# zyang1580/PDA

Measured on AMD Instinct MI355X. Metric: users/sec full-catalogue top-K@50 (eval), higher is better.
Workload: dtype f32; 1 GPU; C3: synthetic 1000000 users x 200000 items, d=128, PDA condition ((elu+1)*pop^0.22) head, masked top-K@50; ranks_seen=1

## Files before the change

include/pda_hip_experimental.h:

```cpp
#ifndef PDA_HIP_EXPERIMENTAL_H
#define PDA_HIP_EXPERIMENTAL_H

#include "pda_hip.h"

#ifdef __cplusplus
extern "C" {
#endif

int pda_score_topk_huge_splits(int n_users_blk, int n_items_local, int d);

int pda_topk_kth_value(const uint64_t* keys, int n_splits, int n_users_blk, int K, int pos, float* out, void* stream);
int pda_topk_remap_items(uint64_t* keys, size_t n_keys, const int32_t* gid, int n_gid, void* stream);
int pda_topk_seed_bounds(const uint64_t* keys, int n_splits, int n_users_blk, int K, int m, float* bounds, void* stream);
int pda_topk_seed_counts(const uint64_t* keys, int n_splits, int n_users_blk, int K, const float* bounds, int n_thr, int32_t* counts,
                         void* stream);
int pda_topk_seed_pick(const float* bounds, const int32_t* counts, int n_thr, int n_users_blk, int K, float* seed, void* stream);
int pda_topk_seed_refine(const uint64_t* keys, int n_splits, int n_users_blk, int K, float* lo, float* hi, float* mid, int32_t* counts,
                         int mode, void* stream);
int pda_score_topk4_phase_f32(const float* U, const float* I_shard, const void* prep, const float* pop_shard, const int32_t* users,
                              int n_users_blk, int item_offset, int n_items_local, int d, const int64_t* hist_indptr,
                              const int32_t* hist_indices, int hist_row_mode, int K, int head, int early_stop, int n_splits,
                              int phase, int warm_tiles, const float* seed, uint64_t* out_keys, void* workspace, void* stream);
int pda_score_topk4_phase_bf16(const uint16_t* U, const uint16_t* I_shard, const void* prep, const float* pop_shard,
                               const int32_t* users, int n_users_blk, int item_offset, int n_items_local, int d,
                               const int64_t* hist_indptr, const int32_t* hist_indices, int hist_row_mode, int K, int head,
                               int early_stop, int n_splits, int phase, int warm_tiles, const float* seed, uint64_t* out_keys,
                               void* workspace, void* stream);
int pda_score_topk4_phase_image_offsets(int n_users_blk, int n_items_local, int d, int n_splits, size_t* offs);
int pda_score_topk4_phase_user_image(const void* U, int bf16, const int32_t* users, int n_users_blk, int d, void* ufrag, float* unorm,
                                     void* stream);
int pda_score_topk4_phase_mask_table(const void* prep, int n_items_local, int d, int item_offset, const int64_t* hist_indptr,
                                     const int32_t* hist_indices, int n_rows, uint32_t* table, void* stream);
int pda_score_topk4_phase_masked_f32(const float* U, const float* I_shard, const void* prep, const float* pop_shard, const int32_t* users,
                                     int n_users_blk, int item_offset, int n_items_local, int d, const int64_t* hist_indptr,
                                     const int32_t* hist_indices, int hist_row_mode, int K, int head, int early_stop, int n_splits,
                                     const uint32_t* mask_table, int mask_table_rows, uint64_t* out_keys, void* workspace, void* stream);
int pda_score_topk4_phase_masked_bf16(const uint16_t* U, const uint16_t* I_shard, const void* prep, const float* pop_shard, const int32_t* users,
                                      int n_users_blk, int item_offset, int n_items_local, int d, const int64_t* hist_indptr,
                                      const int32_t* hist_indices, int hist_row_mode, int K, int head, int early_stop, int n_splits,
                                      const uint32_t* mask_table, int mask_table_rows, uint64_t* out_keys, void* workspace, void* stream);
int pda_score_topk4_phase_mask_rows(const void* prep, const int32_t* users, int n_users_blk, int item_offset, int n_items_local, int d,
                                    const int64_t* hist_indptr, const int32_t* hist_indices, int hist_row_mode, int warm_tiles, uint32_t* out,
                                    void* stream);
int pda_score_topk4_phase_mask_offsets(int n_users_blk, int n_items_local, int d, int n_splits, size_t* offs);
int pda_score_topk7_phase_user_image(const void* U, int bf16, const int32_t* users, int n_users_blk, int d, void* ufrag, float* unorm, float* uerr,
                                     void* stream);
int pda_score_topk4_phase_bloom_rows(const void* prep, const int32_t* users, int n_users_blk, const int64_t* hist_indptr,
                                     const int32_t* hist_indices, int hist_row_mode, int skip_if_ordered, uint32_t* bloom, void* stream);
int pda_score_topk7_phase_bloom_rows(const void* prep, const int32_t* users, int n_users_blk, int item_offset, int n_items_local, int d,
                                     const int64_t* hist_indptr, const int32_t* hist_indices, int hist_row_mode, uint32_t* bloom, void* stream);
#define PDA_SWEEP_WARM_ONE_KERNEL 2048
#define PDA_SWEEP_TAIL_NO_SHARE 4096
#define PDA_SWEEP_TAIL_OTHERS_FIRST 8192
#define PDA_SWEEP_TAIL_MIN2 16384

size_t pda_triplet_plan_bytes(int B);
size_t pda_triplet_plan_large_workspace_bytes(int B);
int pda_triplet_plan_large(const int32_t* users, const int32_t* pos, const int32_t* neg, int B, void* plan, void* workspace, void* stream);
size_t pda_bpr_step_plan_scratch_bytes(int B, int d);
int pda_triplet_plan(const int32_t* users, const int32_t* pos, const int32_t* neg, int B, int n_batches, void* plans, void* stream);
int pda_bpr_step_plan_f32(float* U, float* I, const int32_t* users, const int32_t* pos, const int32_t* neg, const float* pos_pop,
                          const float* neg_pop, int B, int d, float regs, float reg_div, float lr, const void* plan, float* scratch,
                          int exact, float* loss_acc, void* stream);
int pda_bpr_step_plan_bf16(uint16_t* U_bf16, uint16_t* I_bf16, float* U_master, float* I_master, const int32_t* users,
                           const int32_t* pos, const int32_t* neg, const float* pos_pop, const float* neg_pop, int B, int d,
                           float regs, float reg_div, float lr, const void* plan, float* scratch, float* loss_acc, void* stream);

int pda_sort_triplets_by_pos(int32_t* users, int32_t* pos, int32_t* neg, float* pos_pop, float* neg_pop, int B,
                             void* stream);

int pda_group_triplets_by_pos(int32_t* users, int32_t* pos, int32_t* neg, float* pos_pop, float* neg_pop, int B,
                              void* stream);

int pda_adam_mark_rows(const int32_t* users, const int32_t* pos, const int32_t* neg, int B, uint32_t* touched_u, uint32_t* touched_i, void* stream);
int pda_adam_dense_sweep3_f32(float* var_a, float* m_a, float* v_a, float* g_a, size_t rows_a, uint32_t* touched_a, float* var_b, float* m_b, float* v_b,
                              float* g_b, size_t rows_b, uint32_t* touched_b, int d, float lr_t, float beta1, float beta2, float eps, void* stream);

int pda_adam_rows_f32(float* var, float* m, float* v, float* g, const int32_t* rows, int n_rows, int d, float lr_t,
                      float beta1, float beta2, float eps, void* stream);

int pda_adam_lazy_f32(int phase, float* U, float* mU, float* vU, float* gU, int32_t* lastU, float* I, float* mI, float* vI,
                      float* gI, int32_t* lastI, const int32_t* users, const int32_t* pos, const int32_t* neg, int B, int d, int t,
                      const float* lr_tab, float beta1, float beta2, float eps, void* stream);
int pda_adam_lazy_sync_f32(float* var, float* m, float* v, int32_t* last, size_t n_rows, int d, int t, const float* lr_tab,
                           float beta1, float beta2, float eps, void* stream);
int pda_adam_lazy_dev_f32(int phase, float* U, float* mU, float* vU, float* gU, int32_t* lastU, float* I, float* mI, float* vI,
                          float* gI, int32_t* lastI, const int32_t* users, const int32_t* pos, const int32_t* neg, int B, int d,
                          const int32_t* t_dev, int32_t* t_next, const float* lr_tab, int n_tab, float beta1, float beta2, float eps,
                          void* stream);
#define PDA_ADAM_REPLAY_FAST 0x10
int pda_adam_lazy_sync_fast_f32(float* var, float* m, float* v, int32_t* last, size_t n_rows, int d, int t, const float* lr_tab,
                                float beta1, float beta2, float eps, void* stream);

typedef struct pda_sample_job {
    int32_t* users; int gen_users; const int32_t* user_pool; int n_pool; int B;
    const int64_t* train_indptr; const int32_t* train_indices; const int32_t* train_slots;
    int neg_lo, neg_hi; const float* pop_matrix; int n_slots; uint64_t seed;
    const uint64_t* step_dev; uint64_t* step_next;
    int32_t* pos; int32_t* neg; float* pos_pop; float* neg_pop;
} pda_sample_job;
int pda_bpr_step_sample_f32(float* U, float* I, const int32_t* users, const int32_t* pos, const int32_t* neg,
                            const float* pos_pop, const float* neg_pop, int B, int d, float regs, float reg_div, float lr,
                            int update_mode, float* loss_acc, const pda_sample_job* next, void* stream);

int pda_sample_batches_dev(int32_t* users, int gen_users, const int32_t* user_pool, int n_pool, int B, int n_batches,
                           const int64_t* train_indptr, const int32_t* train_indices, const int32_t* train_slots, int neg_lo,
                           int neg_hi, const float* pop_matrix, int n_slots, uint64_t seed, const uint64_t* step_dev,
                           uint64_t* step_next, int32_t* pos, int32_t* neg, float* pos_pop, float* neg_pop, int group_by_pos,
                           void* stream);
int pda_group_triplets_by_pos_batches(int32_t* users, int32_t* pos, int32_t* neg, float* pos_pop, float* neg_pop, int B,
                                      int n_batches, void* stream);

int pda_bpr_train_steps_f32(float* U, float* I, int d, float regs, float reg_div, float lr, int update_mode,
                            const pda_sample_job* set0, const pda_sample_job* set1, uint64_t* step_ctr, int n_steps,
                            float* loss_acc, float* loss_steps, void* barrier_ws, void* stream);

double pda_peak_mfma_flops_per_launch(int iters);
int pda_peak_mfma_bf16(float* sink, int iters, void* stream);
int pda_peak_mfma_bf16_const(float* sink, int iters, void* stream);
double pda_peak_mfma_lds_flops_per_launch(int n_blk);
int pda_peak_mfma_lds_bf16(const void* rows, size_t n_bytes, void* out, int n_blk, void* stream);
int pda_peak_copy(const float* src, float* dst, size_t n_floats, void* stream);

#ifdef __cplusplus
}
#endif
#endif
// ... 1 lines not shown
```

pda_amd/_lib.py:

```python
from __future__ import annotations

import ctypes as C
import os

_HERE = os.path.dirname(os.path.abspath(__file__))
LIB_PATH = os.environ.get("PDA_HIP_LIB") or os.path.join(_HERE, "csrc", "libpda_hip.so")

ABI_VERSION = 2
HEAD_RAW, HEAD_POP = 0, 1
HIST_BY_BLOCK_ROW, HIST_BY_USER_ID = 0, 1
UPD_NONE, UPD_SGD_FUSED, UPD_DENSE_GRAD = 0, 1, 2
UPD_ANY_ORDER = 0x100
UPD_USERS_DISTINCT = 0x200
ADAM_REPLAY_FAST = 0x10
MAX_K = 64
TOPK_CAP = 60

_vp, _i, _f, _u64, _sz = C.c_void_p, C.c_int, C.c_float, C.c_uint64, C.c_size_t

class ScorePlan(C.Structure):
    _fields_ = [("path", _i), ("sweep_mode", _i), ("n_splits", _i), ("early_stop", _i), ("order", _i), ("prep_with_pop", _i),
                ("workspace_bytes", _sz), ("keys_rows", _sz)]


class SampleJob(C.Structure):
    _fields_ = [("users", _vp), ("gen_users", _i), ("user_pool", _vp), ("n_pool", _i), ("B", _i),
                ("train_indptr", _vp), ("train_indices", _vp), ("train_slots", _vp),
                ("neg_lo", _i), ("neg_hi", _i), ("pop_matrix", _vp), ("n_slots", _i), ("seed", _u64),
                ("step_dev", _vp), ("step_next", _vp),
                ("pos", _vp), ("neg", _vp), ("pos_pop", _vp), ("neg_pop", _vp)]


SIGNATURES = {
    "pda_abi_version": (_i, []),
    "pda_error_string": (C.c_char_p, [_i]),
    "pda_score_topk_auto_splits": (_i, [_i, _i]),
    "pda_score_topk_f32": (_i, [_vp, _vp, _vp, _vp, _i, _i, _i, _i, _vp, _vp, _i, _i, _i, _i, _vp, _vp]),
    "pda_item_prep_bytes": (_sz, [_i, _i]),
    "pda_item_prep_f32": (_i, [_vp, _i, _i, _vp, _vp]),
    "pda_score_topk_workspace_bytes": (_sz, [_i]),
    "pda_score_topk4_workspace_bytes": (_sz, [_i, _i, _i, _i]),
    "pda_score_topk_prepped_f32": (_i, [_vp, _vp, _vp, _vp, _vp, _i, _i, _i, _i, _vp, _vp, _i, _i, _i, _i, _vp, _vp, _vp]),
    "pda_item_prep_ordered_bytes": (_sz, [_i, _i]),
    "pda_item_prep_ordered_f32": (_i, [_vp, _vp, _vp, _i, _i, _vp, _vp]),
    "pda_item_prep_ordered_check": (_i, [_vp, _i, _i, _vp]),
    "pda_hist_reorder": (_i, [_vp, _i, _i, _i, _vp, _vp, _i, _vp, _vp]),
    "pda_score_topk_ordered_f32": (_i, [_vp, _vp, _vp, _vp, _vp, _i, _i, _i, _i, _vp, _vp, _vp, _i, _i, _i, _i, _i, _vp, _vp, _vp]),
    "pda_item_prep_bf16_bytes": (_sz, [_i, _i]),
    "pda_item_prep_bf16": (_i, [_vp, _i, _i, _vp, _vp]),
    "pda_score_topk_bf16": (_i, [_vp, _vp, _vp, _vp, _vp, _i, _i, _i, _i, _vp, _vp, _i, _i, _i, _i, _vp, _vp, _vp]),
    "pda_item_prep_ordered_bf16_bytes": (_sz, [_i, _i]),
    "pda_item_prep_ordered_bf16": (_i, [_vp, _vp, _vp, _i, _i, _vp, _vp]),
    "pda_score_topk_ordered_bf16": (_i, [_vp, _vp, _vp, _vp, _vp, _i, _i, _i, _i, _vp, _vp, _vp, _i, _i, _i, _i, _i, _vp, _vp, _vp]),
    "pda_item_prep4_bytes": (_sz, [_i, _i]),
    "pda_item_prep4_f32": (_i, [_vp, _vp, _vp, _i, _i, _vp, _vp]),
    "pda_item_prep4_bf16": (_i, [_vp, _vp, _vp, _i, _i, _vp, _vp]),
    "pda_item_prep7_f32": (_i, [_vp, _vp, _i, _i, _vp, _vp]),
    "pda_item_prep7_bf16": (_i, [_vp, _vp, _i, _i, _vp, _vp]),
    "pda_item_prep4_check": (_i, [_vp, _i, _i, _vp]),
    "pda_score_topk4_auto_splits": (_i, [_i, _i, _i]),
    "pda_score_topk4_f32": (_i, [_vp, _vp, _vp, _vp, _vp, _i, _i, _i, _i, _vp, _vp, _i, _i, _i, _i, _i, _vp, _vp, _vp]),
    "pda_score_topk4_bf16": (_i, [_vp, _vp, _vp, _vp, _vp, _i, _i, _i, _i, _vp, _vp, _i, _i, _i, _i, _i, _vp, _vp, _vp]),
    "pda_peak_mfma_flops_per_launch": (C.c_double, [_i]),
    "pda_peak_mfma_bf16": (_i, [_vp, _i, _vp]),
    "pda_peak_mfma_bf16_const": (_i, [_vp, _i, _vp]),
    "pda_peak_mfma_lds_flops_per_launch": (C.c_double, [_i]),
    "pda_peak_mfma_lds_bf16": (_i, [_vp, _sz, _vp, _i, _vp]),
    "pda_peak_copy": (_i, [_vp, _vp, _sz, _vp]),
    "pda_topk_kth_value": (_i, [_vp, _i, _i, _i, _i, _vp, _vp]),
    "pda_topk_remap_items": (_i, [_vp, _sz, _vp, _i, _vp]),
    "pda_topk_seed_refine": (_i, [_vp, _i, _i, _i, _vp, _vp, _vp, _vp, _i, _vp]),
    "pda_topk_seed_bounds": (_i, [_vp, _i, _i, _i, _i, _vp, _vp]),
    "pda_topk_seed_counts": (_i, [_vp, _i, _i, _i, _vp, _i, _vp, _vp]),
    "pda_topk_seed_pick": (_i, [_vp, _vp, _i, _i, _i, _vp, _vp]),
    "pda_score_topk4_phase_f32": (_i, [_vp, _vp, _vp, _vp, _vp, _i, _i, _i, _i, _vp, _vp, _i, _i, _i, _i, _i, _i, _i, _vp, _vp, _vp, _vp]),
    "pda_score_topk4_phase_bf16": (_i, [_vp, _vp, _vp, _vp, _vp, _i, _i, _i, _i, _vp, _vp, _i, _i, _i, _i, _i, _i, _i, _vp, _vp, _vp, _vp]),
    "pda_score_topk4_phase_image_offsets": (_i, [_i, _i, _i, _i, _vp]),
    "pda_score_topk4_phase_user_image": (_i, [_vp, _i, _vp, _i, _i, _vp, _vp, _vp]),
    "pda_score_topk4_phase_mask_table": (_i, [_vp, _i, _i, _i, _vp, _vp, _i, _vp, _vp]),
    "pda_score_topk4_phase_mask_rows": (_i, [_vp, _vp, _i, _i, _i, _i, _vp, _vp, _i, _i, _vp, _vp]),
    "pda_score_topk4_phase_mask_offsets": (_i, [_i, _i, _i, _i, _vp]),
    "pda_score_topk7_phase_user_image": (_i, [_vp, _i, _vp, _i, _i, _vp, _vp, _vp, _vp]),
    "pda_score_topk4_phase_bloom_rows": (_i, [_vp, _vp, _i, _vp, _vp, _i, _i, _vp, _vp]),
    "pda_score_topk7_phase_bloom_rows": (_i, [_vp, _vp, _i, _i, _i, _i, _vp, _vp, _i, _vp, _vp]),
    "pda_score_topk4_phase_masked_f32": (_i, [_vp, _vp, _vp, _vp, _vp, _i, _i, _i, _i, _vp, _vp, _i, _i, _i, _i, _i, _vp, _i, _vp, _vp, _vp]),
    "pda_score_topk4_phase_masked_bf16": (_i, [_vp, _vp, _vp, _vp, _vp, _i, _i, _i, _i, _vp, _vp, _i, _i, _i, _i, _i, _vp, _i, _vp, _vp, _vp]),
    "pda_score_topk_plan": (_i, [_i, _i, _i, _i, _i, _i, _i, _i, _vp]),
    "pda_score_topk_huge_splits": (_i, [_i, _i, _i]),
    "pda_score_topk7_workspace_bytes": (_sz, [_i, _i, _i]),
    "pda_score_topk7_f32": (_i, [_vp, _vp, _vp, _vp, _i, _i, _i, _i, _vp, _vp, _i, _i, _i, _vp, _vp, _vp]),
    "pda_score_topk7_bf16": (_i, [_vp, _vp, _vp, _vp, _i, _i, _i, _i, _vp, _vp, _i, _i, _i, _vp, _vp, _vp]),
    "pda_topk_merge": (_i, [_vp, _i, _i, _i, _vp, _vp, _vp, _vp, _vp, _vp, _i, _vp]),
    "pda_bpr_step_f32": (_i, [_vp, _vp, _vp, _vp, _vp, _vp, _vp, _i, _i, _f, _f, _f, _i, _vp, _vp, _vp, _vp, _vp, _vp, _vp]),
    "pda_triplet_plan_bytes": (_sz, [_i]),
    "pda_bpr_step_plan_scratch_bytes": (_sz, [_i, _i]),
    "pda_triplet_plan": (_i, [_vp, _vp, _vp, _i, _i, _vp, _vp]),
    "pda_triplet_plan_large_workspace_bytes": (_sz, [_i]),
    "pda_triplet_plan_large": (_i, [_vp, _vp, _vp, _i, _vp, _vp, _vp]),
    "pda_bpr_step_plan_f32": (_i, [_vp, _vp, _vp, _vp, _vp, _vp, _vp, _i, _i, _f, _f, _f, _vp, _vp, _i, _vp, _vp]),
    "pda_bpr_step_plan_bf16": (_i, [_vp, _vp, _vp, _vp, _vp, _vp, _vp, _vp, _vp, _i, _i, _f, _f, _f, _vp, _vp, _vp, _vp]),
    "pda_sgd_apply_f32": (_i, [_vp, _vp, _vp, _vp, _vp, _vp, _vp, _vp, _i, _i, _f, _vp]),
    "pda_bpr_step_shard_f32": (_i, [_vp, _vp, _i, _vp, _vp, _vp, _vp, _vp, _i, _i, _f, _f, _f, _f, _vp, _i, _vp, _vp, _vp]),
    "pda_apply_user_grads_f32": (_i, [_vp, _vp, _vp, _i, _i, _i, _f, _vp]),
    "pda_bpr_step_bf16": (_i, [_vp, _vp, _vp, _vp, _vp, _vp, _vp, _vp, _vp, _i, _i, _f, _f, _f, _i, _vp, _vp, _vp, _vp, _vp, _vp, _vp]),
    "pda_refresh_rows_bf16": (_i, [_vp, _vp, _vp, _i, _i, _vp]),
    "pda_group_triplets_by_pos": (_i, [_vp, _vp, _vp, _vp, _vp, _i, _vp]),
    "pda_sort_triplets_by_pos": (_i, [_vp, _vp, _vp, _vp, _vp, _i, _vp]),
    "pda_adam_dense_sweep_f32": (_i, [_vp, _vp, _vp, _vp, _sz, _f, _f, _f, _f, _vp]),
    "pda_adam_dense_sweep2_f32": (_i, [_vp, _vp, _vp, _vp, _sz, _vp, _vp, _vp, _vp, _sz, _f, _f, _f, _f, _vp]),
    "pda_adam_mark_rows": (_i, [_vp, _vp, _vp, _i, _vp, _vp, _vp]),
    "pda_adam_dense_sweep3_f32": (_i, [_vp, _vp, _vp, _vp, _sz, _vp, _vp, _vp, _vp, _vp, _sz, _vp, _i, _f, _f, _f, _f, _vp]),
    "pda_score_dense_f32": (_i, [_vp, _vp, _vp, _vp, _i, _vp, _i, _i, _i, _vp, _vp]),
    "pda_adam_dense_sweep4_f32": (_i, [_vp, _vp, _vp, _vp, _sz, _vp, _vp, _vp, _vp, _vp, _sz, _vp, _i, _i, _f, _f, _f, _f, _i, _vp]),
    "pda_adam_step_f32": (_i, [_vp, _vp, _vp, _vp, _vp, _sz, _vp, _vp, _vp, _vp, _vp, _sz, _vp, _vp, _vp, _vp, _vp, _i, _i, _f, _f, _i, _f, _f, _f, _f,
                               _i, _i, _vp, _vp]),
    "pda_adam_rows_f32": (_i, [_vp, _vp, _vp, _vp, _vp, _i, _i, _f, _f, _f, _f, _vp]),
    "pda_adam_lazy_f32": (_i, [_i] + [_vp] * 13 + [_i, _i, _i, _vp, _f, _f, _f, _vp]),
    "pda_adam_lazy_dev_f32": (_i, [_i] + [_vp] * 13 + [_i, _i, _vp, _vp, _vp, _i, _f, _f, _f, _vp]),
    "pda_adam_lazy_sync_f32": (_i, [_vp, _vp, _vp, _vp, _sz, _i, _i, _vp, _f, _f, _f, _vp]),
    "pda_adam_lazy_sync_fast_f32": (_i, [_vp, _vp, _vp, _vp, _sz, _i, _i, _vp, _f, _f, _f, _vp]),
    "pda_metrics": (_i, [_vp, _i, _i, _vp, _vp, _vp, _i, _vp, _vp]),
    "pda_sample_triplets_dev": (_i, [_vp, _i, _vp, _i, _i, _vp, _vp, _vp, _i, _i, _vp, _i, _u64, _vp, _vp, _vp, _vp, _vp, _vp, _vp]),
    "pda_sample_batches_dev": (_i, [_vp, _i, _vp, _i, _i, _i, _vp, _vp, _vp, _i, _i, _vp, _i, _u64, _vp, _vp, _vp, _vp, _vp, _vp, _i, _vp]),
    "pda_group_triplets_by_pos_batches": (_i, [_vp, _vp, _vp, _vp, _vp, _i, _i, _vp]),
    "pda_counter_add": (_i, [_vp, _u64, _vp]),
    "pda_bpr_step_sample_f32": (_i, [_vp, _vp, _vp, _vp, _vp, _vp, _vp, _i, _i, _f, _f, _f, _i, _vp, _vp, _vp]),
    "pda_bpr_train_steps_f32": (_i, [_vp, _vp, _i, _f, _f, _f, _i, _vp, _vp, _vp, _i, _vp, _vp, _vp, _vp]),
    "pda_sample_triplets": (_i, [_vp, _i, _vp, _i, _i, _vp, _vp, _vp, _i, _i, _vp, _i, _u64, _u64, _vp, _vp, _vp, _vp, _vp]),
}

HEAD_BIAS = 2
TEMP_POP_SIGNATURES = {
    "pda_temp_pop_step_f32": (_i, [_vp] * 8 + [_i, _i, _i, _f, _f] + [_vp] * 6 + [_i, _vp, _vp]),
    "pda_temp_pop_sweep_f32": (_i, [_vp] * 5 + [_sz] + [_vp] * 5 + [_sz] + [_vp] * 8 + [_i, _i, _i, _f, _f, _f, _f, _vp]),
    "pda_temp_pop_adam_step_f32": (_i, [_vp] * 5 + [_sz] + [_vp] * 5 + [_sz] + [_vp] * 12 + [_i, _i, _i, _f, _f, _i, _f, _f, _f, _f, _vp, _vp]),
    "pda_temp_pop_score_workspace_bytes": (_sz, [_i]),
    "pda_temp_pop_score_topk_f32": (_i, [_vp] * 6 + [_i, _i, _i, _i, _vp, _vp, _i, _i, _i, _vp, _vp, _vp]),
}

HEAD_PC = 3
PC_MAX_K = 50
_d = C.c_double
PC_SIGNATURES = {
    "pda_pc_moments_workspace_bytes": (_sz, [_i, _i]),
    "pda_pc_item_moments_f32": (_i, [_vp, _vp, _i, _i, _vp, _vp, _vp]),
    "pda_pc_user_stats_f32": (_i, [_vp] * 5 + [_i, _i, _i, _vp, _vp, _i, _d, _vp, _vp, _vp, _vp]),
    "pda_pc_score_workspace_bytes": (_sz, [_i, _i, _i, _i]),
    "pda_pc_score_topk_f32": (_i, [_vp] * 5 + [_i, _i, _i, _vp, _vp, _i, _d, _d, _i, _i, _vp, _vp, _vp, _vp]),
}

DET_SIGNATURES = {
    "pda_bpr_grad_plan_scratch_bytes": (_sz, [_i, _i]),
    "pda_bpr_grad_plan_f32": (_i, [_vp] * 7 + [_i, _i, _f, _f] + [_vp] * 6 + [_i, _vp, _vp]),
    "pda_adam_step_plan_f32": (_i, [_vp] * 5 + [_sz] + [_vp] * 5 + [_sz] + [_vp] * 5 + [_i, _i, _f, _f, _i, _f, _f, _f, _f, _i, _vp, _vp, _vp, _vp]),
    "pda_metrics_ordered_workspace_bytes": (_sz, [_i, _i]),
    "pda_metrics_ordered": (_i, [_vp, _i, _i, _vp, _vp, _vp, _i, _vp, _vp, _vp]),
}

DEEP_MAX_K = 1024
DEEP_MERGE_MAX_KEYS = 8192
DEEP_SIGNATURES = {
    "pda_deep_topk_workspace_bytes": (_sz, [_i, _i, _i, _i]),
    "pda_deep_topk_f32": (_i, [_vp] * 4 + [_i, _i, _i, _i, _vp, _vp, _i, _i, _i, _vp, _vp, _vp, _vp, _sz, _vp]),
    "pda_deep_topk_bf16": (_i, [_vp] * 4 + [_i, _i, _i, _i, _vp, _vp, _i, _i, _i, _vp, _vp, _vp, _vp, _sz, _vp]),
    "pda_metrics_deep_workspace_bytes": (_sz, [_i, _i]),
    "pda_metrics_deep": (_i, [_vp, _i, _i, _vp, _vp, _vp, _i, _vp, _vp, _vp]),
    "pda_deep_merge": (_i, [_vp, _i, _i, _i, _vp, _vp, _vp, _vp, _vp, _vp, _i, _vp]),
}

# ... 203 lines not shown
```

pda_amd/csrc/pda_score_topk_v4.hip:

```cpp
#include "pda_v4_shared.h"
#include <cstdlib>
#include <type_traits>

using namespace pda_topk;

namespace {

constexpr int kCap4 = 57;
constexpr int kRing4 = 128;
constexpr int kWarmTiles = 4;
constexpr int kMainWaves = 8;
#ifndef PDA_W4_ABL
#define PDA_W4_ABL 0
#endif
#ifdef PDA_V4_PROF
__device__ unsigned long long pda_prof4[24];
#define PROF_T0(v) const long long v = __builtin_readcyclecounter()
#define PROF_T1(v, slot) prof[slot] += (unsigned long long)(__builtin_readcyclecounter() - v)
#define PROF_INC(slot, x) prof[slot] += (unsigned long long)(x)
#define PROF_FLUSH(first, last) do { if (lane == 0) for (int pq = (first); pq <= (last); ++pq) atomicAdd(&pda_prof4[pq], prof[pq]); } while (0)
#else
#define PROF_T0(v) do {} while (0)
#define PROF_T1(v, slot) do {} while (0)
#define PROF_INC(slot, x) do {} while (0)
#define PROF_FLUSH(first, last) do {} while (0)
#endif
constexpr unsigned kSpinMax = 1u << 26;


struct Args4 {
    const void* U;
    const void* I;
    const float* pop;
    const int32_t* users;
    const int64_t* hist_indptr;
    const int32_t* hist_indices;
    uint64_t* out_keys;
    const unsigned char* rows;
    const float* sufA;
    const float* sufB;
    const int* pos_of;
    unsigned* stats;
    uint64_t* lists_ws;
    int32_t* regroup_ws;
    float* pred_ws;
    const int32_t* row_perm;
    const uint32_t* hmask_ws;
    const uint32_t* bloom;
    const int* prep_hdr;
    const float* seed;
    int n_users_blk, item_offset, n_items_local, hist_row_mode, K, n_splits, n_tiles;
    int warm_tiles;
    int warm_sorted;
    uint64_t* handover;
    const unsigned char* rows5;
    const float* meta5;
    const unsigned char* ufrag;
    const float* unorm;
    int prep_hdr_pop;
    int warm_final;
    int warm_shared;
    float* seed_out;
    const int* n_users_dev;
    int lists_empty;
    const float* tailA;
    const float* tailB;
    unsigned char* ufrag_out;
    float* unorm_out;
    float* kth_ws;
    const uint32_t* hmask_tab;
    int hmask_tab_rows;
    uint32_t* wscore;
    uint64_t* tail_rec;
    unsigned tail_min;
    int tail_others_first;
};

struct Call4 {
    enum Warm { kNoWarm, kWarm4, kWarmTwo };
    enum Sweep { kNoSweep, kSweep4, kSweep4Many, kSweep5 };
    Warm warm;
    bool warm_whole;
    bool mask_kernel;
    bool bloom;
    bool uprep5;
    Sweep sweep;
    bool early_stop;
    bool regroup;
    bool ends_in_warm;
};

constexpr int kMaxDev4 = 64;
int dynamic_lds_once(const void* kernel, size_t bytes, char (&done)[kMaxDev4], int* dev_out = nullptr) {
    int dev = 0;
    if (hipGetDevice(&dev) != hipSuccess || dev < 0 || dev >= kMaxDev4) return PDA_ERR_LAUNCH;
    if (!done[dev]) {
        if (hipFuncSetAttribute(kernel, hipFuncAttributeMaxDynamicSharedMemorySize, (int)bytes) != hipSuccess) return PDA_ERR_LAUNCH;
        done[dev] = 1;
    }
    if (dev_out != nullptr) *dev_out = dev;
    return PDA_OK;
}


template <int D, bool BF>
__global__ void __launch_bounds__(256) prep4_kernel(const void* __restrict__ I, const float* __restrict__ pop, const int* __restrict__ order,
                                                    int n, int n_pad, unsigned char* __restrict__ rows, int* __restrict__ pos_of,
                                                    int* __restrict__ hdr, unsigned char* __restrict__ rows5, int* __restrict__ meta5, u32x4* __restrict__ pinfo,
                                                    int f16img) {
    constexpr int TPR = D / 8, RB = row_bytes(D);
    const int pos = blockIdx.x * (256 / TPR) + threadIdx.x / TPR, e = threadIdx.x % TPR;
    if (pos >= n_pad) return;
    unsigned char* rp = rows + (size_t)pos * RB;
    float ss = 0.f, popv = 1.0f, rs = 0.f;
    int src = -1;
    if (pos < n) {
        src = pos;
        if (order) {
            src = order[pos];
            if (src < 0 || src >= n) { if (e == 0) atomicOr(hdr, 1); src = 0; }
            else if (e == 0 && atomicExch(&pos_of[src], pos) != -1) atomicOr(hdr, 1);
        } else if (e == 0) {
            pos_of[pos] = pos;
        }
        if (pop) popv = pop[src];
        const f32x4 a = pda_load4<BF>(I, (size_t)src * D + 8 * e);
        const f32x4 b = pda_load4<BF>(I, (size_t)src * D + 8 * e + 4);
        u32x4 hq, lq;
        split8(a, b, hq, lq);
        *reinterpret_cast<u32x4*>(rp + 16 * e) = hq;
#pragma unroll
        for (int k = 0; k < 4; ++k) ss += a[k] * a[k] + b[k] * b[k];
        {
            const float pv = pop ? ((popv == popv) ? popv : 0.f) : 1.0f;
            f32x4 as = a, bs = b;
#pragma unroll
            for (int k = 0; k < 4; ++k) { as[k] *= pv; bs[k] *= pv; }
            u32x4 hs, ls;
            if (f16img) {
                hs = pack_half8(as, bs, rs);
            } else {
                split8(as, bs, hs, ls);
#pragma unroll
                for (int k = 0; k < 4; ++k) {
                    const float r0 = as[k] - __uint_as_float((k & 1) ? (hs[k >> 1] & 0xFFFF0000u) : (hs[k >> 1] << 16));
                    const float r1 = bs[k] - __uint_as_float((k & 1) ? (hs[2 + (k >> 1)] & 0xFFFF0000u) : (hs[2 + (k >> 1)] << 16));
                    rs += r0 * r0 + r1 * r1;
                }
            }
            const int r5 = pos & 31;
            const int sw = D >= 128 ? (r5 & 15) : ((r5 >> 1) & 7);
            *reinterpret_cast<u32x4*>(rows5 + (size_t)(pos >> 5) * (64 * D) + r5 * (2 * D) + ((e ^ sw) << 4)) = hs;
        }
    } else {
        const u32x4 z = {0u, 0u, 0u, 0u};
        *reinterpret_cast<u32x4*>(rp + 16 * e) = z;
        {
            const int r5 = pos & 31;
            const int sw = D >= 128 ? (r5 & 15) : ((r5 >> 1) & 7);
// ... 475 lines not shown
            nb = h ? hib : lob;
        };
        int ca_t, cb_t;
        count_ge2(1u, 1u, ca_t, cb_t);
        uint32_t ta = 1u, tb = 1u;
        const bool needa = ca_t > cap_t, needb = cb_t > cap_t;
        if (__any(needa || needb)) {
            uint32_t mxa = 0u, mna = 0xFFFFFFFFu, mxb = 0u, mnb = 0xFFFFFFFFu;
#pragma unroll
            for (int k = 0; k < NHT; ++k) {
                const uint32_t va = ordv[k][r], vb = ordv[k][r + 1];
                mxa = max(mxa, va);
                mna = min(mna, va != 0u ? va : 0xFFFFFFFFu);
                mxb = max(mxb, vb);
                mnb = min(mnb, vb != 0u ? vb : 0xFFFFFFFFu);
            }
#pragma unroll
            for (int o = 16; o >= 1; o >>= 1) {
                mxa = max(mxa, (uint32_t)__shfl_xor((int)mxa, o, 64));
                mna = min(mna, (uint32_t)__shfl_xor((int)mna, o, 64));
                mxb = max(mxb, (uint32_t)__shfl_xor((int)mxb, o, 64));
                mnb = min(mnb, (uint32_t)__shfl_xor((int)mnb, o, 64));
            }
            uint32_t hia = mxa + 1u, hib = mxb + 1u;
            if (needa) ta = mna;
            if (needb) tb = mnb;
            for (int it = 0; it < 40; ++it) {
                const bool opena = needa && ca_t > cap_t && hia - ta > 1u;
                const bool openb = needb && cb_t > cap_t && hib - tb > 1u;
                if (!__any(opena || openb)) break;
                const uint32_t mida = opena ? ta + ((hia - ta) >> 1) : ta;
                const uint32_t midb = openb ? tb + ((hib - tb) >> 1) : tb;
                int cnta, cntb;
                count_ge2(mida, midb, cnta, cntb);
                if (opena) {
                    if (cnta >= K) {
                        ta = mida;
                        ca_t = cnta;
                    } else {
                        hia = mida;
                    }
                }
                if (openb) {
                    if (cntb >= K) {
                        tb = midb;
                        cb_t = cntb;
                    } else {
                        hib = midb;
                    }
                }
            }
        }
        emit_row(r, ta, ca_t);
        emit_row(r + 1, tb, cb_t);
    }
    pda_wave_sync();
    if (tid == 0) atomicAdd(reinterpret_cast<unsigned long long*>(g.stats + 2), (unsigned long long)(2 * nwarm));
    for (int rr = 0; rr < 32; ++rr) {
        uint64_t* buf = my_lists + rr * CAP;
        if (((PDA_W4_ABL & 4) == 0) && (g.warm_sorted || g.warm_final || (g.handover == nullptr && __builtin_amdgcn_readfirstlane(cntl[wave * 32 + rr]) > K)))
            compact_list<CAP>(buf, &cntl[wave * 32 + rr], &taul[wave * 32 + rr], K, lane);
        const int c = cntl[wave * 32 + rr];
        const int rb = utile * kUserTile + wave * 32 + rr;
        if (g.seed_out != nullptr) {
            uint32_t mn = lane < c ? (uint32_t)(buf[lane] >> 32) : 0xFFFFFFFFu;
#pragma unroll
            for (int o = 32; o >= 1; o >>= 1) mn = min(mn, (uint32_t)__shfl_xor((int)mn, o, 64));
            if (lane == 0 && rb < g.n_users_blk) g.seed_out[rb] = c >= K ? pda_unordf(mn) : -INFINITY;
        }
        if (g.kth_ws != nullptr) continue;
        if (g.handover != nullptr) {
            if (rb < g.n_users_blk && lane < CAP) g.handover[((size_t)split * g.n_users_blk + rb) * CAP + lane] = lane < c ? buf[lane] : 0ull;
            if (g.warm_final && rb < g.n_users_blk && lane < K) g.out_keys[((size_t)split * g.n_users_blk + rb) * K + lane] = lane < c ? buf[lane] : 0ull;
        } else if (rb < g.n_users_blk && lane < K) {
            const uint64_t k = lane < c ? buf[lane] : 0ull;
            g.out_keys[((size_t)split * g.n_users_blk + rb) * K + lane] = k;
        }
    }
    if (g.kth_ws != nullptr) {
        pda_wave_sync();
        const int rb0 = utile * kUserTile + wave * 32, nv = max(0, min(32, g.n_users_blk - rb0));
        if (lane < nv) {
            const uint64_t kl = my_lists[(size_t)lane * CAP + (K - 1)];
            g.kth_ws[(size_t)split * g.n_users_blk + rb0 + lane] = cntl[wave * 32 + lane] >= K ? pda_unordf((uint32_t)(kl >> 32)) : -INFINITY;
        }
        uint64_t* ob = g.out_keys + ((size_t)split * g.n_users_blk + rb0) * K;
        const int q64 = 64 / K, r64 = 64 % K;
        int rr = lane / K, p = lane % K;
        for (int i = lane; i < nv * K; i += 64) {
            ob[i] = p < cntl[wave * 32 + rr] ? my_lists[(size_t)rr * CAP + p] : 0ull;
            rr += q64;
            p += r64;
            if (p >= K) { p -= K; ++rr; }
        }
    }
    if (g.pred_ws != nullptr && lane < 32) {
        const int rb = utile * kUserTile + wave * 32 + lane;
        if (rb < g.n_users_blk) {
            g.pred_ws[2 * (size_t)rb] = predt[wave * 32 + lane];
            g.pred_ws[2 * (size_t)rb + 1] = nul[wave * 32 + lane];
        }
    }
}

constexpr int kWS5Waves = 8, kWS5Threads = 64 * kWS5Waves;
constexpr int kWarmPos = 64 * kWarmTiles;
constexpr size_t warm_score5_lds(int d) { return (size_t)kWarmPos * d * 4 + kWarmPos * 8 + (size_t)kWS5Waves * 32 * 2 * kWarmTiles * 4; }

template <int D, bool BF>
__global__ void __launch_bounds__(kWS5Threads) warm_score5_kernel(Args4 g) {
    extern __shared__ __attribute__((aligned(16))) unsigned char smem[];
    constexpr int RB = row_bytes(D);
    constexpr int NC = D / 8;
    constexpr int CPR4 = D / 4;
    float* Bt = reinterpret_cast<float*>(smem);
    float* popw = Bt + kWarmPos * D;
    int* idw = reinterpret_cast<int*>(popw + kWarmPos);
    unsigned* hmask = reinterpret_cast<unsigned*>(idw + kWarmPos);

    const int tid = threadIdx.x, lane = tid & 63, wave = tid >> 6;
    const int j = lane & 31, h = lane >> 5;
    const int nwarm = g.warm_tiles;
    const int npos = 64 * nwarm;
    for (int p = tid; p < npos; p += kWS5Threads) {
        const float* tl = reinterpret_cast<const float*>(g.rows + (size_t)p * RB + 2 * D + 32);
        popw[p] = tl[0];
        idw[p] = reinterpret_cast<const int*>(tl)[1];
    }
    __syncthreads();
    for (int id = tid; id < npos * CPR4; id += kWS5Threads) {
        const int jj = id / CPR4, ch = id % CPR4;
        *reinterpret_cast<f32x4*>(Bt + jj * D + 4 * (ch ^ swz<D>(jj & 31))) = pda_load4<BF>(g.I, (size_t)idw[jj] * D + 4 * ch);
    }
    if (blockIdx.x == 0) {
        for (int p = tid; p < kWarmPos; p += kWS5Threads) g.wscore[p] = p < npos ? (uint32_t)idw[p] : 0u;
        if (tid == 0) g.stats[8] = 5u;
    }
    __syncthreads();

    uint32_t* scores = g.wscore + kWarmPos;
    const int utiles_w = (g.n_users_blk + kUserTile - 1) / kUserTile;
    const int nunits = utiles_w * (kUserTile / 32);
    const int G = (int)gridDim.x, stride = G * kWS5Waves;
    unsigned* hm_l = hmask + wave * 32 * 2 * kWarmTiles;
    static_assert(2 * kWarmTiles == 8, "two 16-byte loads per row");

    auto row_uid = [&](int unit) -> int {
        const int rb = unit * 32 + j;
        return (unit < nunits && rb < g.n_users_blk) ? g.users[rb] : 0;
    };
    auto load_rows = [&](int unit_x, int uid, f32x4 (&a)[NC], u32x4& hm, bool& hm_on) __attribute__((always_inline)) {
        if (unit_x >= nunits) return;
        const int rb = unit_x * 32 + j;
#pragma unroll
        for (int c = 0; c < NC; ++c) a[c] = pda_load4<BF>(g.U, (size_t)uid * D + 4 * h + 8 * c);
        hm_on = false;
        if (g.hmask_tab != nullptr) {
            hm_on = rb < g.n_users_blk && (unsigned)uid < (unsigned)g.hmask_tab_rows;
            hm = *reinterpret_cast<const u32x4*>(g.hmask_tab + (size_t)(hm_on ? uid : 0) * (2 * kWarmTiles) + 4 * h);
        } else if (g.hmask_ws != nullptr) {
            hm_on = true;
            hm = *reinterpret_cast<const u32x4*>(g.hmask_ws + (size_t)rb * (2 * kWarmTiles) + 4 * h);
        }
    };
    unsigned long long n_tiles_done = 0ull;
    auto run_unit = [&](const int unit_in, f32x4 (&areg)[NC], const u32x4& hm_in, const bool hm_on) __attribute__((always_inline)) {
        const int unit = __builtin_amdgcn_readfirstlane(unit_in);
        const int row_blk = unit * 32 + j;
        if (unit * 32 + 32 > g.n_users_blk) {
            const f32x4 z = {0.f, 0.f, 0.f, 0.f};
#pragma unroll
            for (int c = 0; c < NC; ++c) areg[c] = row_blk < g.n_users_blk ? areg[c] : z;
        }
        const u32x4 hz = {0u, 0u, 0u, 0u};
        const u32x4 hmv = hm_on ? hm_in : hz;
        *reinterpret_cast<u32x4*>(hm_l + j * (2 * kWarmTiles) + 4 * h) = hmv;
// ... 147 lines not shown
            t[s] = 1u;
            hi[s] = 0u;
            need[s] = ct[s] > CAP;
        }
        if (need[0] || need[1]) {
#pragma unroll
            for (int s = 0; s < 2; ++s) {
                uint32_t mx = max(max(v[s][0], v[s][1]), max(v[s][2], v[s][3])), mn = 0xFFFFFFFFu;
#pragma unroll
                for (int q = 0; q < 4; ++q) mn = min(mn, v[s][q] != 0u ? v[s][q] : 0xFFFFFFFFu);
#pragma unroll
                for (int o = 32; o >= 1; o >>= 1) {
                    mx = max(mx, (uint32_t)__shfl_xor((int)mx, o, 64));
                    mn = min(mn, (uint32_t)__shfl_xor((int)mn, o, 64));
                }
                hi[s] = (uint32_t)__builtin_amdgcn_readfirstlane((int)mx) + 1u;
                if (need[s]) t[s] = (uint32_t)__builtin_amdgcn_readfirstlane((int)mn);
            }
            for (int step = 0; step < 40; ++step) {
                const bool open0 = need[0] && ct[0] > CAP && hi[0] - t[0] > 1u;
                const bool open1 = need[1] && ct[1] > CAP && hi[1] - t[1] > 1u;
                if (!(open0 || open1)) break;
                const uint32_t mid0 = open0 ? t[0] + ((hi[0] - t[0]) >> 1) : t[0];
                const uint32_t mid1 = open1 ? t[1] + ((hi[1] - t[1]) >> 1) : t[1];
                const int c0 = count32(v[0], mid0), c1 = count32(v[1], mid1);
                if (open0) {
                    if (c0 >= K) { t[0] = mid0; ct[0] = c0; } else { hi[0] = mid0; }
                }
                if (open1) {
                    if (c1 >= K) { t[1] = mid1; ct[1] = c1; } else { hi[1] = mid1; }
                }
            }
        }
        uint64_t thr[2];
#pragma unroll
        for (int s = 0; s < 2; ++s) {
            thr[s] = (uint64_t)t[s] << 32;
            if (ct[s] > CAP) {
                uint64_t lo64 = thr[s], hi64 = (uint64_t)(t[s] + 1u) << 32;
                for (int step = 0; step < 40 && ct[s] > CAP && hi64 - lo64 > 1ull; ++step) {
                    const uint64_t mid = lo64 + ((hi64 - lo64) >> 1);
                    const int c = count64(v[s], mid);
                    if (c >= K) { lo64 = mid; ct[s] = c; } else { hi64 = mid; }
                }
                thr[s] = lo64;
            }
        }
        int cs[2];
#pragma unroll
        for (int s = 0; s < 2; ++s) {
            uint64_t* buf = lists[wave][s];
            int run = 0;
#pragma unroll
            for (int q = 0; q < 4; ++q) {
                const uint64_t key = key_of(v[s], q);
                const bool p = key >= thr[s];
                const uint64_t bm = __ballot(p);
                const int slot = run + (int)__builtin_amdgcn_mbcnt_hi((uint32_t)(bm >> 32), __builtin_amdgcn_mbcnt_lo((uint32_t)bm, 0));
                if (p && slot < 64) buf[slot] = key;
                run += __popcll(bm);
            }
            cs[s] = min(run, CAP);
            if (lane >= cs[s]) buf[lane] = 0ull;
        }
        pda_wave_sync();
        uint64_t key[2];
        int rank[2] = {0, 0};
        key[0] = lists[wave][0][lane];
        key[1] = lists[wave][1][lane];
        const int cm = max(cs[0], cs[1]);
        for (int jj = 0; jj < cm; jj += 4) {
#pragma unroll
            for (int s = 0; s < 2; ++s) {
                const uint64_t* buf = lists[wave][s];
                const uint64_t k0 = buf[jj], k1 = buf[jj + 1], k2 = buf[jj + 2], k3 = buf[jj + 3];
                rank[s] += ((k0 > key[s]) ? 1 : 0) + ((k1 > key[s]) ? 1 : 0) + ((k2 > key[s]) ? 1 : 0) + ((k3 > key[s]) ? 1 : 0);
            }
        }
        pda_wave_sync();
#pragma unroll
        for (int s = 0; s < 2; ++s)
            if (lane < cs[s]) lists[wave][s][rank[s]] = key[s];
        pda_wave_sync();
#pragma unroll
        for (int s = 0; s < 2; ++s) {
            const int rb = rb0 + it + s;
            if (rb < n) {
                if (lane < K) g.out_keys[(size_t)rb * K + lane] = lists[wave][s][lane];
                const uint64_t kl = lists[wave][s][K - 1];
                if (lane == it + s) kth_mine = cs[s] >= K ? pda_unordf((uint32_t)(kl >> 32)) : -INFINITY;
            }
        }
        pda_wave_sync();
    }
    if (lane < kSelRows && rb0 + lane < n) {
        g.kth_ws[rb0 + lane] = kth_mine;
        if (g.seed_out != nullptr) g.seed_out[rb0 + lane] = kth_mine;
    }
}


#include "pda_v4_block_asm.h"
constexpr int kPF4 = 4;
constexpr int kRSleep4 = 8;
constexpr int kLSleep4 = 1;
constexpr int kRingMany4 = 128;
constexpr int kLoaders256 = 3;
constexpr int kNB256 = 2;
constexpr int kNSlotMax4 = 5;
constexpr int kNSlot4 = 4;
template <int D, int GM = 0>
struct Geo4 {
    static_assert(GM == 0 || GM == 3, "geometries: 0 = default, 3 = many candidates");
    static constexpr bool MANY = D <= 128 && GM == 3;
    static constexpr int MW = MANY ? 4 : kMainWaves;
    static constexpr int UA = 1;
    static constexpr bool GL = D > 128;
    static constexpr int NB = D <= 128 ? 2 : kNB256;
    static constexpr int LOADERS = D <= 128 ? 4 : kLoaders256;
    static constexpr int RESCORERS = MANY ? 8 : (D <= 128 ? 4 : 4 - kLoaders256);
    static constexpr int ROWS = 32 * UA;
    static constexpr int NRINGS = MW > RESCORERS ? MW : RESCORERS;
    static constexpr int RPW = NRINGS / MW;
    static constexpr int RPR = ROWS / RPW;
    static constexpr int MPR = NRINGS / RESCORERS;
    static constexpr int WAVES = MW + LOADERS + RESCORERS;
    static constexpr int UT = MW * ROWS;
    static constexpr int RB = row_bytes(D), TB = tile_bytes(D);
    static constexpr int HB = 32 * RB;
    static constexpr int BB = NB * HB;
    static constexpr int NP = (BB + 1023) / 1024;
    static constexpr int LASTL = (BB % 1024) ? (BB % 1024) / 16 : 64;
    static constexpr int NSLOT = (GL || MANY) ? kNSlot4 : 2;
    static constexpr size_t lds_tiles = NSLOT * (size_t)BB;
    static constexpr int CAP = MANY ? 64 : kCap4;
    static constexpr size_t lds_lists = GL ? 0 : (size_t)UT * CAP * 8;
    static constexpr int RING = MANY ? kRingMany4 : kRing4;
    static constexpr size_t lds_total = lds_tiles + lds_lists + (size_t)UT * 8 + kMainWaves * RING * 4 + 512;
    static_assert(NRINGS <= kMainWaves && RPW * MW == NRINGS && MPR * RESCORERS == NRINGS, "ring bookkeeping: eight words each");
    static_assert(NSLOT >= 2 && NSLOT <= kNSlotMax4, "vote timing of the early termination");
};

template <int D, int HEAD, bool BF, bool ES, int GM = 0>
__global__ void __launch_bounds__((64 * Geo4<D, GM>::WAVES)) sweep4_kernel(Args4 g) {
    using G = Geo4<D, GM>;
    constexpr int kLoaders = G::LOADERS, kMPR = G::MPR, MW = G::MW, RPW = G::RPW, RPR = G::RPR;
    constexpr int NB = G::NB, ROWS = G::ROWS, UT = G::UT, RB = G::RB, HB = G::HB, BB = G::BB, NP = G::NP, UA = G::UA, NSLOT = G::NSLOT;
    constexpr bool GL = G::GL;
    constexpr int CAPL = G::CAP;
    constexpr int RINGL = G::RING;
    constexpr int NM = D / 16;
    constexpr float kEps = BF ? 6.103515625e-5f : 7.890625e-3f;
    extern __shared__ __attribute__((aligned(16))) unsigned char smem[];
    unsigned char* tiles = smem;
    uint64_t* lists = GL ? g.lists_ws + (size_t)blockIdx.x * UT * CAPL
                         : reinterpret_cast<uint64_t*>(smem + G::lds_tiles);
    int* cntl = reinterpret_cast<int*>(smem + G::lds_tiles + G::lds_lists);
    float* taul = reinterpret_cast<float*>(cntl + UT);
    unsigned* rings = reinterpret_cast<unsigned*>(taul + UT);
    unsigned* sync = rings + kMainWaves * RINGL;
    unsigned* s_landed = sync;
    unsigned* s_stop = sync + 108;
    unsigned* s_released = sync + 4;
    unsigned* s_tail = sync + 12;
    unsigned* s_head = sync + 20;
    unsigned* s_done = sync + 28;
    unsigned* s_tver = sync + 36;
    unsigned* s_vote = sync + 44;
    unsigned* s_uns = sync + 112;

    const int tid = threadIdx.x, lane = tid & 63;
    const int wave = __builtin_amdgcn_readfirstlane(tid >> 6);
    const int split = blockIdx.x % g.n_splits, utile = blockIdx.x / g.n_splits;
    if (g.n_users_dev != nullptr && utile * UT >= *g.n_users_dev) return;
    const int K = g.K;
    const int nt = split_tiles(g.n_tiles, split, g.n_splits);
    const int wt = warm_tiles_of(g, split);
    const bool starts_empty = g.lists_empty || (g.warm_shared && split > 0);
    const int n_it = max(0, nt - wt);
    const int n_blk = NB > 2 ? (2 * n_it) / NB : n_it * (2 / NB);
// ... 891 lines not shown
        if (c.warm == Call4::kWarmTwo) {
            constexpr size_t smem = warm_score5_lds(D);
            static char attr_done[kMaxDev4] = {};
            static int cu_of_dev[kMaxDev4] = {};
            int dev = 0;
            if (const int rc = dynamic_lds_once(reinterpret_cast<const void*>(&warm_score5_kernel<D, BF>), smem, attr_done, &dev)) return rc;
            if (cu_of_dev[dev] == 0) {
                int cus = 0;
                if (hipDeviceGetAttribute(&cus, hipDeviceAttributeMultiprocessorCount, dev) != hipSuccess || cus <= 0) return PDA_ERR_LAUNCH;
                cu_of_dev[dev] = cus;
            }
            const int n_cu = cu_of_dev[dev];
            const int nunits = utiles * (kUserTile / 32);
            hipLaunchKernelGGL((warm_score5_kernel<D, BF>), dim3((unsigned)(n_cu < nunits ? n_cu : nunits)), dim3(kWS5Threads), smem, stream, gw);
            PDA_CHECK_LAUNCH();
            hipLaunchKernelGGL(warm_select5_kernel, dim3((unsigned)((g.n_users_blk + 4 * kSelRows - 1) / (4 * kSelRows))), dim3(256), 0, stream, gw);
            PDA_CHECK_LAUNCH();
            return PDA_OK;
        }
    }
    if (c.warm != Call4::kWarm4) return PDA_ERR_ARG;
    constexpr size_t smem = 32 * D * 4 + (size_t)kUserTile * (kCap4 * 8 + 8) + kUserTile * 2 * kWarmTiles * 4 + 256 + kUserTile * 8;
    static char attr_done[kMaxDev4] = {};
    if (const int rc = dynamic_lds_once(reinterpret_cast<const void*>(&warm4_kernel<D, HEAD, BF>), smem, attr_done)) return rc;
    hipLaunchKernelGGL((warm4_kernel<D, HEAD, BF>), dim3((unsigned)(utiles * gw.n_splits)), dim3(kThreads), smem, stream, gw);
    PDA_CHECK_LAUNCH();
    return PDA_OK;
}

template <int D, int HEAD, bool BF>
int launch4(const Args4& g, const Call4& c, hipStream_t stream) {
    if (c.warm != Call4::kNoWarm) {
        if (const int rc = launch_warm4<D, HEAD, BF>(g, c, stream)) return rc;
    }
    if (c.sweep == Call4::kNoSweep || c.ends_in_warm) return PDA_OK;
    if constexpr (HEAD == PDA_HEAD_POP) {
        if (c.sweep == Call4::kSweep5) return launch_sweep5<D, BF, true, D == 256 ? 128 : 256>(g, c, stream);
    }
    if constexpr (D <= 128) {
        if (c.sweep == Call4::kSweep4Many) return launch_sweep4<D, HEAD, BF, 3>(g, c, stream);
    }
    if (c.sweep != Call4::kSweep4) return PDA_ERR_ARG;
    return launch_sweep4<D, HEAD, BF, 0>(g, c, stream);
}

int user_tile4(int d) { return d == 64 ? Geo4<64>::UT : d == 128 ? Geo4<128>::UT : Geo4<256>::UT; }
struct Ws4 {
    size_t tailrec, lists, bloom, hmask, regroup, handover, ufrag, unorm, seed, kth, wscore, total;
};
static Ws4 ws4_layout(int n_users_blk, int d, int n_splits) {
    auto al = [](size_t x) { return (x + 255) & ~(size_t)255; };
    Ws4 w{};
    w.tailrec = al(pda_score_topk_workspace_bytes(n_users_blk));
    w.lists = al(w.tailrec + ((size_t)n_users_blk + 511) / 512 * (size_t)n_splits * 8);
    size_t b = w.lists;
    const size_t ut = 1024;
    b += ((size_t)n_users_blk + ut - 1) / ut * (size_t)n_splits * ut * kCap4 * 8 + 256;
    w.bloom = al(b);
    w.hmask = al(w.bloom + (size_t)n_users_blk * 128);
    w.regroup = al(w.hmask + ((size_t)n_users_blk + kUserTile - 1) / kUserTile * (size_t)n_splits * kUserTile * 2 * kWarmTiles * 4);
    w.handover = al(w.regroup + (1024 + 4 * (size_t)n_users_blk) * 4);
    w.total = w.handover + (size_t)n_splits * (size_t)n_users_blk * kCap4 * 8;
    w.ufrag = al(w.total);
    w.unorm = w.ufrag;
    {
        const size_t n_pad = ((size_t)n_users_blk + kUT5 - 1) / kUT5 * kUT5;
        w.unorm = w.ufrag + al(n_pad * 2 * (size_t)d);
        w.total = w.unorm + al(n_pad * 4);
    }
    w.seed = w.total;
    w.total = w.seed + al((size_t)n_users_blk * 4);
    w.kth = w.total;
    w.total = w.kth + al((size_t)n_splits * (size_t)n_users_blk * 4);
    w.wscore = w.total;
    w.total = w.wscore + al((size_t)kWarmPos * 4 + ((size_t)n_users_blk + kUserTile - 1) / kUserTile * kUserTile * kWarmPos * 4);
    return w;
}
extern "C" size_t pda_score_topk4_workspace_bytes(int n_users_blk, int n_items_local, int d, int n_splits) {
    if (n_users_blk <= 0 || n_items_local <= 0 || (d != 64 && d != 128 && d != 256)) return 0;
    if (n_splits <= 0) n_splits = pda_score_topk4_auto_splits(n_users_blk, n_items_local, d);
    return ws4_layout(n_users_blk, d, n_splits).total;
}

int run_score4(const void* U, const void* I_shard, bool bf16, const void* prep, const float* pop_shard, const int32_t* users,
               int n_users_blk, int item_offset, int n_items_local, int d, const int64_t* hist_indptr, const int32_t* hist_indices,
               int hist_row_mode, int K, int head, int early_stop, int n_splits, uint64_t* out_keys, void* workspace, hipStream_t s,
               int phase = 3, const float* seed = nullptr, int warm_tiles = 0, const int* n_users_dev = nullptr,
               const uint32_t* mask_table = nullptr, int mask_table_rows = 0) {
    if (!U || !I_shard || !prep || !users || !out_keys || !workspace) return PDA_ERR_ARG;
    if (n_users_blk <= 0 || n_items_local <= 0 || item_offset < 0) return PDA_ERR_ARG;
    if (K < 1 || K > PDA_MAX_K) return PDA_ERR_ARG;
    if (early_stop < 0 || (early_stop & ~0x7FFF) != 0) return PDA_ERR_ARG;
    const bool warm_per_split = (early_stop & PDA_SWEEP_WARM_PER_SPLIT) != 0;
    const bool warm_one_kernel = (early_stop & PDA_SWEEP_WARM_ONE_KERNEL) != 0;
    const bool tail_share = (early_stop & PDA_SWEEP_TAIL_NO_SHARE) == 0;
    const bool tail_others_first = (early_stop & PDA_SWEEP_TAIL_OTHERS_FIRST) != 0, tail_min2 = (early_stop & PDA_SWEEP_TAIL_MIN2) != 0;
    int geometry = (early_stop & PDA_SWEEP_HUGE) ? 4 : (early_stop & PDA_SWEEP_MANY_CANDIDATES) ? 3 : 0;
    if (warm_tiles == 0) warm_tiles = (early_stop >> 4) & 7;
    early_stop &= 1;
    if (head != PDA_HEAD_RAW && head != PDA_HEAD_POP) return PDA_ERR_ARG;
    if (head == PDA_HEAD_POP && !pop_shard) return PDA_ERR_ARG;
    if (hist_indptr && !hist_indices) return PDA_ERR_ARG;
    if (d != 64 && d != 128 && d != 256) return PDA_ERR_UNSUPPORTED;
    if (K > kCap4 - 3) return PDA_ERR_UNSUPPORTED;
    if ((uint64_t)n_items_local > (1ull << 26)) return PDA_ERR_UNSUPPORTED;
    if (warm_tiles < 0 || warm_tiles > kWarmTiles) return PDA_ERR_ARG;
    if (warm_tiles == 0) warm_tiles = kWarmTiles;
    const bool from_empty = phase == 4;
    if (from_empty) {
        if (seed == nullptr) return PDA_ERR_ARG;
        phase = 2;
        warm_tiles = 0;
    } else if (phase < 1 || phase > 3) {
        return PDA_ERR_ARG;
    }
    if (n_splits <= 0) n_splits = pda_score_topk4_auto_splits(n_users_blk, n_items_local, d);
    const Prep4Layout L = prep4_layout(n_items_local, d);
    const bool pop_head = head == PDA_HEAD_POP;
    const bool hist = hist_indptr != nullptr;

    Call4 c{};
    c.ends_in_warm = (L.n_tiles + n_splits - 1) / n_splits <= warm_tiles;
    c.early_stop = early_stop != 0;
    c.sweep = !(phase & 2) ? Call4::kNoSweep
              : (geometry == 4 && pop_head && !early_stop) ? Call4::kSweep5
              : (geometry == 3 && d <= 128) ? Call4::kSweep4Many : Call4::kSweep4;
    const bool dense5 = phase == 3 && c.sweep == Call4::kSweep5 && !c.ends_in_warm;
    c.uprep5 = !(dense5 && n_users_dev == nullptr);
    const bool warm_shared = phase == 3 && n_splits > 1 && seed == nullptr && !warm_per_split && L.n_tiles > n_splits * warm_tiles;
    c.warm_whole = n_splits == 1 || warm_shared;
    c.warm = !(phase & 1) ? Call4::kNoWarm
             : (!c.uprep5 && d <= 128 && !warm_one_kernel && c.warm_whole && n_users_blk <= (1 << 21)) ? Call4::kWarmTwo : Call4::kWarm4;
    c.bloom = hist && (c.sweep == Call4::kSweep4 || c.sweep == Call4::kSweep4Many);
    const bool mask_from_table = mask_table != nullptr && hist && hist_row_mode == PDA_HIST_BY_USER_ID && (phase & 1) && n_users_dev == nullptr && c.warm_whole;
    c.mask_kernel = !mask_from_table && hist && (phase & 1) && (n_users_blk >= 98304 || c.warm == Call4::kWarmTwo);
    constexpr int kRegroupMin = 98304;
    c.regroup = early_stop && (phase & 2) && n_splits == 1 && n_users_blk >= kRegroupMin;

    const unsigned char* pb = reinterpret_cast<const unsigned char*>(prep);
    unsigned char* wsb = reinterpret_cast<unsigned char*>(workspace);
    const Ws4 W = ws4_layout(n_users_blk, d, n_splits);
    Args4 g{};
    g.U = U;
    g.I = I_shard;
    g.pop = pop_shard;
    g.users = users;
    g.hist_indptr = hist_indptr;
    g.hist_indices = hist_indices;
    g.out_keys = out_keys;
    g.rows = pb + L.rows;
    g.sufA = early_stop ? reinterpret_cast<const float*>(pb + L.sufA) : nullptr;
    g.sufB = early_stop ? reinterpret_cast<const float*>(pb + (pop_head ? L.sufB : L.sufR)) : nullptr;
    g.pos_of = reinterpret_cast<const int*>(pb + L.pos_of);
    g.stats = reinterpret_cast<unsigned*>(workspace);
    g.lists_ws = reinterpret_cast<uint64_t*>(wsb + W.lists);
    g.prep_hdr = reinterpret_cast<const int*>(pb + L.hdr);
    g.seed = seed;
    g.n_users_blk = n_users_blk;
    g.item_offset = item_offset;
    g.n_items_local = n_items_local;
    g.hist_row_mode = hist_row_mode;
    g.K = K;
    g.n_splits = n_splits;
    g.n_tiles = L.n_tiles;
    g.warm_tiles = warm_tiles;
    g.warm_sorted = (phase == 1 || c.ends_in_warm) ? 1 : 0;
    g.rows5 = pb + L.rows5;
    g.meta5 = reinterpret_cast<const float*>(pb + L.meta5);
    g.ufrag = wsb + W.ufrag;
    g.unorm = reinterpret_cast<const float*>(wsb + W.unorm);
    g.prep_hdr_pop = pop_head ? 1 : 0;
    g.lists_empty = from_empty ? 1 : 0;
    g.n_users_dev = n_users_dev;
    if (dense5) {
        g.warm_final = 1;
        g.kth_ws = reinterpret_cast<float*>(wsb + W.kth);
    } else if (phase == 3 && !c.ends_in_warm) {
        g.handover = reinterpret_cast<uint64_t*>(wsb + W.handover);
    }
    if (!c.uprep5) {
        g.ufrag_out = wsb + W.ufrag;
        g.unorm_out = reinterpret_cast<float*>(wsb + W.unorm);
    }
    if (pop_head) {
        g.tailA = reinterpret_cast<const float*>(pb + L.sufA);
        g.tailB = reinterpret_cast<const float*>(pb + L.sufB);
    }
    if (warm_shared) {
        g.warm_shared = 1;
        g.seed_out = reinterpret_cast<float*>(wsb + W.seed);
        g.seed = g.seed_out;
    }
    const bool counters_reset = (phase & 1) || from_empty;
    constexpr int kTailShareMinHalfTiles = 2048;
    const bool tail_long = 2 * (L.n_tiles / n_splits) >= kTailShareMinHalfTiles || tail_min2 || tail_others_first;
    if (c.sweep == Call4::kSweep5 && tail_share && counters_reset && tail_long) {
        g.tail_rec = reinterpret_cast<uint64_t*>(wsb + W.tailrec);
        g.tail_min = tail_min2 ? 2u : kTailMinChunk;
        g.tail_others_first = tail_others_first ? 1 : 0;
    }
    if (c.warm == Call4::kWarmTwo) g.wscore = reinterpret_cast<uint32_t*>(wsb + W.wscore);
    if (c.bloom) g.bloom = reinterpret_cast<uint32_t*>(wsb + W.bloom);
    if (mask_from_table) {
        g.hmask_tab = mask_table;
        g.hmask_tab_rows = mask_table_rows;
    }
    if (c.mask_kernel) g.hmask_ws = reinterpret_cast<uint32_t*>(wsb + W.hmask);
    if (c.regroup) {
        g.regroup_ws = reinterpret_cast<int32_t*>(wsb + W.regroup);
        if (phase & 1) g.pred_ws = reinterpret_cast<float*>(g.regroup_ws + 1024 + 2 * (size_t)n_users_blk);
    }

    if (counters_reset && hipMemsetAsync(workspace, 0, W.lists, s) != hipSuccess) return PDA_ERR_LAUNCH;
    if (c.bloom) {
        hipLaunchKernelGGL(hist_bloom4_kernel, dim3((unsigned)((n_users_blk + 31) / 32)), dim3(256), 0, s, users, hist_indptr, hist_indices,
                           hist_row_mode, n_users_blk, const_cast<uint32_t*>(g.bloom), g.prep_hdr, pop_head ? 1 : 0);
        PDA_CHECK_LAUNCH();
    }
#define PDA_V4_(DD, BFV) (pop_head ? launch4<DD, PDA_HEAD_POP, BFV>(g, c, s) : launch4<DD, PDA_HEAD_RAW, BFV>(g, c, s))
    switch (d) {
        case 64: return bf16 ? PDA_V4_(64, true) : PDA_V4_(64, false);
        case 128: return bf16 ? PDA_V4_(128, true) : PDA_V4_(128, false);
        case 256: return bf16 ? PDA_V4_(256, true) : PDA_V4_(256, false);
        default: return PDA_ERR_UNSUPPORTED;
    }
#undef PDA_V4_
}

__global__ void __launch_bounds__(256) kth_value_kernel(const uint64_t* __restrict__ keys, int S, int n_users, int K, int pos, float* __restrict__ out) {
    const int u = blockIdx.x * 256 + threadIdx.x;
    if (u >= n_users) return;
    float best = -INFINITY;
// ... 169 lines not shown
}
extern "C" int pda_item_prep7_bf16(const uint16_t* I_shard, const int32_t* order, int n_items_local, int d, void* prep, void* stream) {
    if (!I_shard || !prep || !order || n_items_local <= 0) return PDA_ERR_ARG;
    return run_prep4(I_shard, true, nullptr, order, n_items_local, d, prep, reinterpret_cast<hipStream_t>(stream), 1);
}
extern "C" int pda_item_prep4_check(const void* prep, int n_items_local, int d, void* stream) {
    if (!prep || n_items_local <= 0) return PDA_ERR_ARG;
    int bad = 0;
    hipStream_t s = reinterpret_cast<hipStream_t>(stream);
    if (hipMemcpyAsync(&bad, prep, 4, hipMemcpyDeviceToHost, s) != hipSuccess) return PDA_ERR_LAUNCH;
    if (hipStreamSynchronize(s) != hipSuccess) return PDA_ERR_LAUNCH;
    return bad ? PDA_ERR_ARG : PDA_OK;
}

extern "C" int pda_topk_kth_value(const uint64_t* keys, int n_splits, int n_users_blk, int K, int pos, float* out, void* stream) {
    if (!keys || !out || n_splits < 1 || n_users_blk < 1 || K < 1 || pos < 0 || pos >= K) return PDA_ERR_ARG;
    hipLaunchKernelGGL(kth_value_kernel, dim3((unsigned)((n_users_blk + 255) / 256)), dim3(256), 0, reinterpret_cast<hipStream_t>(stream), keys,
                       n_splits, n_users_blk, K, pos, out);
    PDA_CHECK_LAUNCH();
    return PDA_OK;
}

extern "C" int pda_topk_seed_refine(const uint64_t* keys, int n_splits, int n_users_blk, int K, float* lo, float* hi, float* mid,
                                    int32_t* counts, int mode, void* stream) {
    if (!keys || !lo || !hi || !mid || !counts || n_splits < 1 || n_users_blk < 1 || K < 1 || mode < 0 || mode > 2) return PDA_ERR_ARG;
    hipLaunchKernelGGL(seed_refine_kernel, dim3((unsigned)((n_users_blk + 255) / 256)), dim3(256), 0, reinterpret_cast<hipStream_t>(stream), keys,
                       n_splits, n_users_blk, K, lo, hi, mid, counts, mode);
    PDA_CHECK_LAUNCH();
    return PDA_OK;
}

extern "C" int pda_score_topk4_phase_f32(const float* U, const float* I_shard, const void* prep, const float* pop_shard, const int32_t* users,
                                         int n_users_blk, int item_offset, int n_items_local, int d, const int64_t* hist_indptr,
                                         const int32_t* hist_indices, int hist_row_mode, int K, int head, int early_stop, int n_splits,
                                         int phase, int warm_tiles, const float* seed, uint64_t* out_keys, void* workspace, void* stream) {
    if (phase != 1 && phase != 2 && phase != 4) return PDA_ERR_ARG;
    return run_score4(U, I_shard, false, prep, pop_shard, users, n_users_blk, item_offset, n_items_local, d, hist_indptr, hist_indices,
                      hist_row_mode, K, head, early_stop, n_splits, out_keys, workspace, reinterpret_cast<hipStream_t>(stream), phase, seed, warm_tiles);
}
extern "C" int pda_score_topk4_phase_bf16(const uint16_t* U, const uint16_t* I_shard, const void* prep, const float* pop_shard,
                                          const int32_t* users, int n_users_blk, int item_offset, int n_items_local, int d,
                                          const int64_t* hist_indptr, const int32_t* hist_indices, int hist_row_mode, int K, int head,
                                          int early_stop, int n_splits, int phase, int warm_tiles, const float* seed, uint64_t* out_keys,
                                          void* workspace, void* stream) {
    if (phase != 1 && phase != 2 && phase != 4) return PDA_ERR_ARG;
    return run_score4(U, I_shard, true, prep, pop_shard, users, n_users_blk, item_offset, n_items_local, d, hist_indptr, hist_indices,
                      hist_row_mode, K, head, early_stop, n_splits, out_keys, workspace, reinterpret_cast<hipStream_t>(stream), phase, seed, warm_tiles);
}

extern "C" int pda_score_topk4_f32(const float* U, const float* I_shard, const void* prep, const float* pop_shard, const int32_t* users,
                                   int n_users_blk, int item_offset, int n_items_local, int d, const int64_t* hist_indptr,
                                   const int32_t* hist_indices, int hist_row_mode, int K, int head, int early_stop, int n_splits,
                                   uint64_t* out_keys, void* workspace, void* stream) {
    return run_score4(U, I_shard, false, prep, pop_shard, users, n_users_blk, item_offset, n_items_local, d, hist_indptr, hist_indices,
                      hist_row_mode, K, head, early_stop, n_splits, out_keys, workspace, reinterpret_cast<hipStream_t>(stream));
}
extern "C" int pda_score_topk4_bf16(const uint16_t* U, const uint16_t* I_shard, const void* prep, const float* pop_shard, const int32_t* users,
                                    int n_users_blk, int item_offset, int n_items_local, int d, const int64_t* hist_indptr,
                                    const int32_t* hist_indices, int hist_row_mode, int K, int head, int early_stop, int n_splits,
                                    uint64_t* out_keys, void* workspace, void* stream) {
    return run_score4(U, I_shard, true, prep, pop_shard, users, n_users_blk, item_offset, n_items_local, d, hist_indptr, hist_indices,
                      hist_row_mode, K, head, early_stop, n_splits, out_keys, workspace, reinterpret_cast<hipStream_t>(stream));
}

extern "C" int pda_score_topk4_phase_masked_f32(const float* U, const float* I_shard, const void* prep, const float* pop_shard, const int32_t* users,
                                                int n_users_blk, int item_offset, int n_items_local, int d, const int64_t* hist_indptr,
                                                const int32_t* hist_indices, int hist_row_mode, int K, int head, int early_stop, int n_splits,
                                                const uint32_t* mask_table, int mask_table_rows, uint64_t* out_keys, void* workspace, void* stream) {
    if (mask_table != nullptr && mask_table_rows <= 0) return PDA_ERR_ARG;
    return run_score4(U, I_shard, false, prep, pop_shard, users, n_users_blk, item_offset, n_items_local, d, hist_indptr, hist_indices,
                      hist_row_mode, K, head, early_stop, n_splits, out_keys, workspace, reinterpret_cast<hipStream_t>(stream), 3, nullptr, 0, nullptr,
                      mask_table, mask_table_rows);
}
extern "C" int pda_score_topk4_phase_masked_bf16(const uint16_t* U, const uint16_t* I_shard, const void* prep, const float* pop_shard, const int32_t* users,
                                                 int n_users_blk, int item_offset, int n_items_local, int d, const int64_t* hist_indptr,
                                                 const int32_t* hist_indices, int hist_row_mode, int K, int head, int early_stop, int n_splits,
                                                 const uint32_t* mask_table, int mask_table_rows, uint64_t* out_keys, void* workspace, void* stream) {
    if (mask_table != nullptr && mask_table_rows <= 0) return PDA_ERR_ARG;
    return run_score4(U, I_shard, true, prep, pop_shard, users, n_users_blk, item_offset, n_items_local, d, hist_indptr, hist_indices,
                      hist_row_mode, K, head, early_stop, n_splits, out_keys, workspace, reinterpret_cast<hipStream_t>(stream), 3, nullptr, 0, nullptr,
                      mask_table, mask_table_rows);
}

static Args4 mask_args4(const void* prep, const int32_t* users, int n_rows, int item_offset, int n_items_local, int d, const int64_t* hist_indptr,
                        const int32_t* hist_indices, int hist_row_mode, int warm_tiles) {
    const Prep4Layout L = prep4_layout(n_items_local, d);
    const unsigned char* pb = reinterpret_cast<const unsigned char*>(prep);
    Args4 g{};
    g.users = users;
    g.hist_indptr = hist_indptr;
    g.hist_indices = hist_indices;
    g.pos_of = reinterpret_cast<const int*>(pb + L.pos_of);
    g.n_users_blk = n_rows;
    g.item_offset = item_offset;
    g.n_items_local = n_items_local;
    g.hist_row_mode = hist_row_mode;
    g.n_splits = 1;
    g.n_tiles = L.n_tiles;
    g.warm_tiles = warm_tiles;
    return g;
}
extern "C" int pda_score_topk4_phase_mask_table(const void* prep, int n_items_local, int d, int item_offset, const int64_t* hist_indptr,
                                                const int32_t* hist_indices, int n_rows, uint32_t* table, void* stream) {
    if (!prep || !hist_indptr || !hist_indices || !table || n_rows <= 0 || n_items_local <= 0 || item_offset < 0) return PDA_ERR_ARG;
    if (d != 64 && d != 128 && d != 256) return PDA_ERR_UNSUPPORTED;
    const Args4 g = mask_args4(prep, nullptr, n_rows, item_offset, n_items_local, d, hist_indptr, hist_indices, PDA_HIST_BY_BLOCK_ROW, kWarmTiles);
    hipLaunchKernelGGL(warm_mask_table4_kernel, dim3((unsigned)((n_rows + kUserTile - 1) / kUserTile)), dim3(kThreads), 0, reinterpret_cast<hipStream_t>(stream), g, table);
    PDA_CHECK_LAUNCH();
    return PDA_OK;
}
extern "C" int pda_score_topk4_phase_mask_rows(const void* prep, const int32_t* users, int n_users_blk, int item_offset, int n_items_local, int d,
                                               const int64_t* hist_indptr, const int32_t* hist_indices, int hist_row_mode, int warm_tiles, uint32_t* out,
                                               void* stream) {
    if (!prep || !users || !hist_indptr || !hist_indices || !out || n_users_blk <= 0 || n_items_local <= 0 || item_offset < 0) return PDA_ERR_ARG;
    if (warm_tiles < 1 || warm_tiles > kWarmTiles) return PDA_ERR_ARG;
    if (d != 64 && d != 128 && d != 256) return PDA_ERR_UNSUPPORTED;
    const Args4 g = mask_args4(prep, users, n_users_blk, item_offset, n_items_local, d, hist_indptr, hist_indices, hist_row_mode, warm_tiles);
    hipLaunchKernelGGL(warm_mask4_kernel, dim3((unsigned)((n_users_blk + kUserTile - 1) / kUserTile)), dim3(kThreads), 0, reinterpret_cast<hipStream_t>(stream), g, out);
    PDA_CHECK_LAUNCH();
    return PDA_OK;
}
extern "C" int pda_score_topk4_phase_mask_offsets(int n_users_blk, int n_items_local, int d, int n_splits, size_t* offs) {
    if (n_users_blk <= 0 || n_items_local <= 0 || (d != 64 && d != 128 && d != 256) || !offs) return PDA_ERR_ARG;
    if (n_splits <= 0) n_splits = pda_score_topk4_auto_splits(n_users_blk, n_items_local, d);
    const Ws4 W = ws4_layout(n_users_blk, d, n_splits);
    offs[0] = W.hmask;
    offs[1] = W.regroup - W.hmask;
    return PDA_OK;
}

extern "C" int pda_score_topk4_phase_image_offsets(int n_users_blk, int n_items_local, int d, int n_splits, size_t* offs) {
    if (n_users_blk <= 0 || n_items_local <= 0 || (d != 64 && d != 128 && d != 256) || !offs) return PDA_ERR_ARG;
    if (n_splits <= 0) n_splits = pda_score_topk4_auto_splits(n_users_blk, n_items_local, d);
    const Ws4 W = ws4_layout(n_users_blk, d, n_splits);
    const size_t ut = d == 256 ? 512 : kUT5;
    offs[0] = W.ufrag;
    offs[1] = W.unorm;
    offs[2] = W.kth;
    offs[3] = ((size_t)n_users_blk + ut - 1) / ut * ut;
    return PDA_OK;
}
extern "C" int pda_score_topk4_phase_user_image(const void* U, int bf16, const int32_t* users, int n_users_blk, int d, void* ufrag, float* unorm,
                                                void* stream) {
    if (!U || !users || !ufrag || !unorm || n_users_blk <= 0) return PDA_ERR_ARG;
    if (d != 64 && d != 128 && d != 256) return PDA_ERR_UNSUPPORTED;
    hipStream_t s = reinterpret_cast<hipStream_t>(stream);
    const size_t ut = d == 256 ? 512 : kUT5, n_pad = ((size_t)n_users_blk + ut - 1) / ut * ut;
#define PDA_UIMG_(DD, BFV, UPWV)                                                                                                                \
    hipLaunchKernelGGL((uprep5_kernel<DD, BFV, true, UPWV>), dim3((unsigned)((n_pad * (DD / 8) + 255) / 256)), dim3(256), 0, s, U, users, n_users_blk, \
                       (int)n_pad, reinterpret_cast<unsigned char*>(ufrag), unorm)
    if (d == 64) { if (bf16) PDA_UIMG_(64, true, 256); else PDA_UIMG_(64, false, 256); }
    else if (d == 128) { if (bf16) PDA_UIMG_(128, true, 256); else PDA_UIMG_(128, false, 256); }
    else { if (bf16) PDA_UIMG_(256, true, 128); else PDA_UIMG_(256, false, 128); }
#undef PDA_UIMG_
    PDA_CHECK_LAUNCH();
    return PDA_OK;
}
extern "C" int pda_score_topk4_phase_bloom_rows(const void* prep, const int32_t* users, int n_users_blk, const int64_t* hist_indptr,
                                                const int32_t* hist_indices, int hist_row_mode, int skip_if_ordered, uint32_t* bloom, void* stream) {
    if (!prep || !users || !hist_indptr || !hist_indices || !bloom || n_users_blk <= 0) return PDA_ERR_ARG;
    if (hist_row_mode != PDA_HIST_BY_USER_ID && hist_row_mode != PDA_HIST_BY_BLOCK_ROW) return PDA_ERR_ARG;
    hipLaunchKernelGGL(hist_bloom4_kernel, dim3((unsigned)((n_users_blk + 31) / 32)), dim3(256), 0, reinterpret_cast<hipStream_t>(stream), users, hist_indptr,
                       hist_indices, hist_row_mode, n_users_blk, bloom, reinterpret_cast<const int*>(prep), skip_if_ordered ? 1 : 0);
    PDA_CHECK_LAUNCH();
    return PDA_OK;
}
// ... 1 lines not shown
```

pda_amd/csrc/pda_v5_sweep.h:

```cpp
#pragma once
#ifdef PDA_V6_LOOP_HEADER
#include PDA_V6_LOOP_HEADER
#else
#include "pda_v6_loop_asm.h"
#endif
#include "pda_v6_free_asm.h"
#include "pda_tail_share.h"

#ifdef PDA_V5_EXITPROF
constexpr int kXpMaxWg = 4096, kXpWords = 12;
__device__ unsigned long long pda_v5_exitprof[kXpMaxWg * 4 * kXpWords];
__device__ int pda_v5_tail_pieces;
#define XP(...) __VA_ARGS__
#else
#define XP(...)
#endif
constexpr int kRing5 = 192;



template <int D, bool BF, bool S16, int UPW>
__global__ void __launch_bounds__(256, 1) sweep5_kernel(Args4 g) {
    static_assert(slot_bytes5(D) == Loop6<D, 8>::kSlotBytes, "one LDS image for all loops");
    static_assert(S16, "the loop on v_mfma_f32_32x32x16_bf16 (round 4's first form: 9.16 against 8.07 ms, profiles/README.md) left with round 5; the parameter keeps the kernel's name");
    static_assert((D <= 128 && UPW == 256) || (D == 256 && UPW == 128), "users per wave: 256, or (d = 256) 128 -- 8 blocks x 8 k-steps = 256 AGPRs, one 512-user workgroup per CU");
    constexpr int NK = D / 32, UBW = 16, NU = UPW / UBW;
    constexpr int SS = slot_bytes5(D), UT = 4 * UPW, CAPL = kCap4, RB4 = row_bytes(D);
    constexpr int LPC = D / 32, CPP = 64 / LPC;
    constexpr float kEps5 = BF ? 4.0234375e-3f : 8.046875e-3f;
    extern __shared__ __attribute__((aligned(16))) unsigned char smem[];
    unsigned char* tiles = smem;
    int* cntl = reinterpret_cast<int*>(smem + kNSlot5 * SS);
    float* taul = reinterpret_cast<float*>(cntl + UT);
    uint64_t* crings = reinterpret_cast<uint64_t*>(taul + UT);
    unsigned* sync = reinterpret_cast<unsigned*>(crings + 4 * kRing5);
    unsigned* s_uns = sync + 8;
    unsigned* touched = sync + 40;
    const int tid = threadIdx.x, lane = tid & 63;
    const int wave = __builtin_amdgcn_readfirstlane(tid >> 6);
    const int split = blockIdx.x % g.n_splits, utile = blockIdx.x / g.n_splits;
    XP(unsigned long long xp[kXpWords] = {0, 0, 0, 0, 0, 0, 0, 0, 0, 0, 0, 0}; const unsigned long long xp_k0 = wall_clock64(); unsigned long long xp_out = 0, xp_re = 0;)
    uint64_t* lists = g.handover != nullptr ? g.handover + ((size_t)split * g.n_users_blk + (size_t)utile * UT) * kCap4
                                            : g.lists_ws + (size_t)blockIdx.x * UT * CAPL;
    const int K = g.K;
    const int nt = split_tiles(g.n_tiles, split, g.n_splits);
    const int wt = warm_tiles_of(g, split);
    const bool starts_empty = g.lists_empty || (g.warm_shared && split > 0);
    const bool warm_final = g.warm_final && !starts_empty;
    const int n_it = max(0, nt - wt);
    const unsigned hend = 2u * (unsigned)n_it;
    if (tid < 72) sync[tid] = (tid < 8 || tid >= 40 || warm_final || starts_empty) ? 0u : 0xFFFFFFFFu;
    if (tid == 0 && blockIdx.x == 0) g.stats[4] = (4u << 28) | (4u << 8) | (1u << 13) | ((BF ? 1u : 0u) << 14) | (unsigned)(D >> 6);
    if (starts_empty) {
        for (int rr = tid; rr < UT; rr += 256) {
            cntl[rr] = 0;
            taul[rr] = utile * UT + rr < g.n_users_blk ? -INFINITY : INFINITY;
        }
        __builtin_amdgcn_fence(__ATOMIC_RELEASE, "workgroup");
    } else if (warm_final && g.kth_ws != nullptr) {
        for (int rr = tid; rr < UT; rr += 256) {
            const int rb = utile * UT + rr;
            int c = 0;
            float tau = INFINITY;
            if (rb < g.n_users_blk) {
                tau = g.kth_ws[(size_t)split * g.n_users_blk + rb];
                c = K;
                if (tau == -INFINITY) {
                    const uint64_t* row = g.out_keys + ((size_t)split * g.n_users_blk + rb) * K;
                    for (c = 0; c < K && row[c] != 0ull; ++c) {}
                }
            }
            cntl[rr] = c;
            taul[rr] = tau;
        }
        __builtin_amdgcn_fence(__ATOMIC_RELEASE, "workgroup");
    } else if (warm_final) {
        for (int rr = tid; rr < UT; rr += 256) {
            const int rb = utile * UT + rr;
            int c = 0;
            float tau = INFINITY;
            if (rb < g.n_users_blk) {
                const uint64_t kl = lists[(size_t)rr * CAPL + (K - 1)];
                c = K;
                tau = pda_unordf((uint32_t)(kl >> 32));
                if (kl == 0ull) {
                    tau = -INFINITY;
                    for (c = 0; c < K - 1 && lists[(size_t)rr * CAPL + c] != 0ull; ++c) {}
                }
            }
            cntl[rr] = c;
            taul[rr] = tau;
        }
        __builtin_amdgcn_fence(__ATOMIC_RELEASE, "workgroup");
    } else
    {
        constexpr int NW = 4, PB = 8;
        for (int r0 = wave; r0 < UT; r0 += PB * NW) {
            uint64_t keyv[PB];
#pragma unroll
            for (int q = 0; q < PB; ++q) {
                const int rr = r0 + q * NW, rb = utile * UT + rr;
                keyv[q] = (rr >= UT || rb >= g.n_users_blk) ? 0ull
                          : g.handover != nullptr ? (lane < kCap4 ? g.handover[((size_t)split * g.n_users_blk + rb) * kCap4 + lane] : 0ull)
                          : (lane < K ? g.out_keys[((size_t)split * g.n_users_blk + rb) * K + lane] : 0ull);
            }
#pragma unroll
            for (int q = 0; q < PB; ++q) {
                const int rr = r0 + q * NW;
                if (rr >= UT) break;
                const int rb = utile * UT + rr;
                const uint64_t key = keyv[q];
                const int c = __popcll(__ballot(key != 0ull));
                if (g.handover == nullptr && lane < K) lists[(size_t)rr * CAPL + lane] = key;
                uint32_t mn = key != 0ull ? (uint32_t)(key >> 32) : 0xFFFFFFFFu;
#pragma unroll
                for (int o = 32; o >= 1; o >>= 1) mn = min(mn, (uint32_t)__shfl_xor((int)mn, o, 64));
                if (lane == 0) {
                    cntl[rr] = c;
                    taul[rr] = rb < g.n_users_blk ? (c >= K ? pda_unordf(mn) : -INFINITY) : INFINITY;
                }
            }
        }
        __builtin_amdgcn_fence(__ATOMIC_RELEASE, "workgroup");
    }
    __syncthreads();

    unsigned* bcast = sync + 80;
    uint64_t* const my_rec = g.tail_rec != nullptr ? g.tail_rec + blockIdx.x : nullptr;
    const unsigned lane16 = (unsigned)lane * 16u;
    const unsigned ring_lds = (unsigned)(size_t)(__attribute__((address_space(3))) unsigned char*)tiles;
    unsigned tail_fixed = 0;
    unsigned own_a = 0, own_b = 0;
    auto next_chunk = [&](bool own, bool first, unsigned& vb, unsigned& a, unsigned& b) __attribute__((always_inline)) -> bool {
        if (wave == 0) {
            unsigned ca = 0, cb = 0, cv = blockIdx.x;
            if (own) {
                if (lane == 0 && !pda_ts_claim(my_rec, first, g.tail_min, tail_fixed, ca, cb)) ca = cb = 0;
            } else {
                for (;;) {
                    unsigned long long key = pda_ts_pick(g.tail_rec, gridDim.x, blockIdx.x, (unsigned)lane, 64u);
#pragma unroll
                    for (int o = 32; o >= 1; o >>= 1) { const unsigned long long k2 = __shfl_xor(key, o, 64); key = k2 > key ? k2 : key; }
                    if ((key >> 32) == 0ull) break;
                    bool ok = false;
                    if (lane == 0) ok = pda_ts_steal(g.tail_rec, key, g.tail_min, cv, ca, cb);
                    if (__any(ok)) break;
                    ca = cb = 0;
                }
            }
            if (lane == 0) { bcast[0] = ca; bcast[1] = cb; bcast[2] = cv; }
// ... 65 lines not shown
                    hb = g.hist_indptr[hr];
                    he = g.hist_indptr[hr + 1];
                }
                auto fma8 = [&](float acc, int cq) __attribute__((always_inline)) -> float {
#pragma unroll
                    for (int sidx = 0; sidx < 4; ++sidx) {
                        acc = __builtin_fmaf(uu[2 * cq][sidx], ii[2 * cq][sidx], acc);
                        acc = __builtin_fmaf(uu[2 * cq + 1][sidx], ii[2 * cq + 1][sidx], acc);
                    }
                    return acc;
                };
                float o = 0.f, o_other = 0.f;
                if constexpr (LPC == 8) {
                    float c0 = 0.f, c1 = 0.f, o0 = 0.f, o1 = 0.f;
#pragma unroll
                    for (int ph = 0; ph < LPC; ++ph) {
                        o0 = c0;
                        o1 = c1;
#pragma unroll
                        for (int cc = 0; cc < 4; ++cc) {
#pragma unroll
                            for (int sidx = 0; sidx < 4; ++sidx) {
                                if (cc & 1) {
                                    o1 = __builtin_fmaf(uu[2 * cc][sidx], ii[2 * cc][sidx], o1);
                                    o1 = __builtin_fmaf(uu[2 * cc + 1][sidx], ii[2 * cc + 1][sidx], o1);
                                } else {
                                    o0 = __builtin_fmaf(uu[2 * cc][sidx], ii[2 * cc][sidx], o0);
                                    o0 = __builtin_fmaf(uu[2 * cc + 1][sidx], ii[2 * cc + 1][sidx], o0);
                                }
                            }
                        }
                        if (ph < LPC - 1) {
                            const float r0 = __shfl_up(o0, 1, 64), r1 = __shfl_up(o1, 1, 64);
                            if (q == ph + 1) {
                                c0 = r0;
                                c1 = r1;
                            }
                        }
                    }
                    o = o1;
                    o_other = o0;
                } else if constexpr (LPC == 4) {
                    const bool hi = q >= 2;
                    auto swap2 = [](float x) __attribute__((always_inline)) -> float {
                        return __int_as_float(__builtin_amdgcn_mov_dpp(__float_as_int(x), 0x4E, 0xF, 0xF, true));
                    };
#pragma unroll
                    for (int cq = 0; cq < 4; ++cq) {
                        const float a = fma8(o, cq);
                        const float a_sw = swap2(a);
                        const float b = fma8(hi ? a_sw : o, cq);
                        const float b_sw = swap2(b);
                        o = hi ? b : b_sw;
                    }
                } else {
                    static_assert(LPC == 2, "d = 64");
#pragma unroll
                    for (int cq = 0; cq < 4; ++cq) o = fma8(o, cq);
                }
                const float o0 = LPC == 8 ? o_other : __int_as_float(__builtin_amdgcn_mov_dpp(__float_as_int(o), 0xB1, 0xF, 0xF, true));
                float sc = o0 + o;
                sc = (sc > 0.0f ? sc + 1.0f : __expf(sc)) * pv;
                const float tt = (valid && q == LPC - 1) ? sc : -INFINITY;
                const int item = g.item_offset + loc;
                bool p = valid && q == LPC - 1 && (tt >= fmaxf(c_tau, c_sd));
                if (hist_on && p) {
                    long long lo = hb, hi2 = he;
                    while (lo < hi2) {
                        const long long mid = (lo + hi2) >> 1;
                        if (g.hist_indices[mid] < item) lo = mid + 1; else hi2 = mid;
                    }
                    if (lo < he && g.hist_indices[lo] == item) p = false;
                }
                const uint64_t key = pda_pack_key(tt, (uint32_t)item);
                bool first = false;
                if (p) first = (atomicOr(&touched[(row0 + row) >> 5], 1u << ((row0 + row) & 31)) & (1u << ((row0 + row) & 31))) == 0u;
                if (lazy_rows) {
                    uint64_t need = __ballot(first);
                    if (need != 0ull) {
                        while (need != 0ull) {
                            const int lr = row0 + __builtin_amdgcn_readlane(row, __builtin_ctzll(need));
                            need &= need - 1ull;
                            const int c_r = cntl[lr];
                            if (lane < c_r) lists[(size_t)lr * CAPL + lane] = g.out_keys[((size_t)split * g.n_users_blk + (size_t)(utile * UT + lr)) * K + lane];
                        }
                        list_sync<true>();
                    }
                }
                append_keys<CAPL, true>(p, row0 + row, tt, key, lists, cntl, taul, row0, UPW, K, lane, s_uns);
            }
            n_cand += ring_n;
            ring_n = 0;
        };
        auto extract2 = [&](unsigned hx, unsigned hl) __attribute__((always_inline)) {
            const bool on0 = hx >= 2u && hx - 2u < hl, on1 = hx >= 1u && hx - 1u < hl;
            if (!on0 && !on1) return;
            constexpr int NR = 8, BU = D == 256 ? 2 : 4, NB = NU / BU, NF = BU * NK;
            static_assert(NU % BU == 0 && 2 * BU * NR <= 64, "the masks of a batch: one 64-bit word per lane");
            const unsigned f0 = on0 ? hx - 2u : hx - 1u, f1 = on1 ? hx - 1u : hx - 2u;
            auto item_of = [&](int r) __attribute__((always_inline)) -> unsigned {
                return 16u * (r >> 2) + 4u * hh + (r & 3);
            };
            unsigned pos00 = 0, pos01 = 0;
            float ctv[2], pmx[2];
            const unsigned char* tbv[2];
#pragma unroll
            for (int t = 0; t < 2; ++t) {
                const unsigned ft = t ? f1 : f0;
                const unsigned T = t0 + (ft >> 1) * (unsigned)g.n_splits;
                if (t) pos01 = T * 64u + (ft & 1u) * 32u; else pos00 = T * 64u + (ft & 1u) * 32u;
                const float2 mt = *reinterpret_cast<const float2*>(g.meta5 + 4 * (size_t)(2u * T + (ft & 1u)));
                ctv[t] = __builtin_fmaf(eu, mt.y, mt.x);
                pmx[t] = mt.x;
                tbv[t] = tiles + (ft & (kNSlot5 - 1)) * SS + j * (2 * D);
            }
            constexpr bool AF_ONCE = D == 64;
            u32x4 af[AF_ONCE ? 2 : 1][2 * NK];
            auto load_af = [&](int t) __attribute__((always_inline)) {
#pragma unroll
                for (int ib = 0; ib < 2; ++ib)
#pragma unroll
                    for (int k = 0; k < NK; ++k)
                        af[AF_ONCE ? t : 0][ib * NK + k] = *reinterpret_cast<const u32x4*>(tbv[t] + ib * 16 * (2 * D) + (((4 * k + hh) ^ swz5<D>(j)) << 4));
            };
            unsigned l16 = lane16;
            asm volatile("" : "+v"(l16));
            u32x4 cur[NF];
            auto load_cur = [&](int b) __attribute__((always_inline)) {
                const unsigned char* pb = my_ufrag + (size_t)b * (NF * 1024);
#pragma unroll
                for (int i = 0; i < NF; ++i) cur[i] = *reinterpret_cast<const u32x4*>(pb + (size_t)(l16 + (unsigned)(i >> 2) * 4096u) + (i & 3) * 1024);
            };
            if constexpr (AF_ONCE) {
                load_af(0);
                load_af(1);
            }
            load_cur(0);
#pragma unroll 1
            for (int b = 0; b < NB; ++b) {
                float tlv[BU];
#pragma unroll
                for (int ub = 0; ub < BU; ++ub) tlv[ub] = thr_of(b * BU + ub);
                uint64_t mm = 0ull;
#pragma unroll
                for (int t = 0; t < 2; ++t) {
                    if constexpr (!AF_ONCE) load_af(t);
#pragma unroll
                    for (int ub = 0; ub < BU; ++ub) {
                        const float tl = tlv[ub];
                        const bool clampy = pmx[t] > tl;
                        uint32_t m = 0;
#pragma unroll
                        for (int ib = 0; ib < 2; ++ib) {
                            f32x4 acc = {0.f, 0.f, 0.f, 0.f};
#pragma unroll
                            for (int k = 0; k < NK; ++k)
                                acc = __builtin_amdgcn_mfma_f32_16x16x32_bf16(__builtin_bit_cast(bf16x8, af[AF_ONCE ? t : 0][ib * NK + k]), __builtin_bit_cast(bf16x8, cur[ub * NK + k]), acc, 0, 0, 0);
#pragma unroll
                            for (int r = 0; r < 4; ++r) m |= (acc[r] + ctv[t] > tl) ? (1u << (4 * ib + r)) : 0u;
                        }
                        if (__any(clampy)) {
#pragma unroll
                            for (int r = 0; r < NR; ++r) {
                                const unsigned pp = (t ? pos01 : pos00) + item_of(r);
                                const float pi = clampy ? *reinterpret_cast<const float*>(g.rows + (size_t)pp * RB4 + 2 * D + 32) : 0.f;
                                m |= (clampy && pi > tl) ? (1u << r) : 0u;
                            }
// ... 55 lines not shown
                }
                lo = __builtin_amdgcn_readfirstlane(lo);
                hi = __builtin_amdgcn_readfirstlane(hi);
            }
            return 2u * (unsigned)lo;
#endif
        };
        float* xch = reinterpret_cast<float*>(sync + 72);
        unsigned h = 0, issued = 0, n_entries = 0;
        unsigned hlim = hend;
        bool hend_ok = true;
        if ((ring_lds & (D == 256 ? 511u : 255u)) != 0u) { if (lane == 0) g.stats[0] = 6u; hend_ok = false; }
        for (unsigned guard = 0; hend_ok && guard < 2u * hend + 8u; ++guard) {
            float thr[NU];
#pragma unroll
            for (int u = 0; u < NU; ++u) thr[u] = thr_of(u);
            unsigned reason = 0;
            float tmin = thr[0];
#pragma unroll
            for (int u = 1; u < NU; ++u) tmin = fminf(tmin, thr[u]);
#pragma unroll
            for (int o = 32; o >= 1; o >>= 1) tmin = fminf(tmin, __shfl_xor(tmin, o, 64));
            tmin = __int_as_float(__builtin_amdgcn_readfirstlane(__float_as_int(tmin)));
            if (lane == 0) { xch[wave] = tmin; xch[4 + wave] = numax; }
            __syncthreads();
            const float tw = __int_as_float(__builtin_amdgcn_readfirstlane(__float_as_int(fminf(fminf(xch[0], xch[1]), fminf(xch[2], xch[3])))));
            const float nw = __int_as_float(__builtin_amdgcn_readfirstlane(__float_as_int(fmaxf(fmaxf(xch[4], xch[5]), fmaxf(xch[6], xch[7])))));
            const unsigned hf = decided(tw, nw, h);
            if (h >= min(hlim, hf)) {
                if (h > hlim) h = hlim;
                if (issued > hlim) issued = hlim;
                if (h < hend) {
                    XP(if (xp_out != 0) { const unsigned long long t_ = wall_clock64(); xp[3] += t_ - xp_out; xp[2] += t_ - xp_re; xp_out = 0; } else xp[6] = wall_clock64() - xp_k0;
                       xp[8] = h; xp[9] = wall_clock64() - xp_k0;)
                    own_a = h;
                    own_b = hend;
                    if (my_rec != nullptr && tid == 0) pda_ts_publish(my_rec, h, hend);
                }
                break;
            }
            hlim = min(hlim, hf);
            ++n_entries;
            XP(if (xp_out != 0) { const unsigned long long t_ = wall_clock64(); xp[3] += t_ - xp_out; xp[2] += t_ - xp_re; } else xp[6] = wall_clock64() - xp_k0;)
            Loop6<D, NU>::run(h, issued, reason, hlim, ring_lds, flags_lds, 1024u * (unsigned)wave, t0, (unsigned)g.n_splits,
                              (unsigned)img, (unsigned)(img >> 32), (unsigned)meta, (unsigned)(meta >> 32), eu, tmin, my_ufrag, thr, lane16);
            XP(xp_out = wall_clock64(); xp_re = xp_out;)
            if (reason == 0u) {
                if (hlim == hend) break;
                continue;
            }
            if (reason != 1u) { if (lane == 0) g.stats[0] = 5u; break; }
            [[maybe_unused]] const unsigned before = ring_n + n_cand;
            extract2(h, hlim);
            XP(const unsigned long long xp_a = wall_clock64(); xp[0] += xp_a - xp_out; xp[4] += 1;)
            if (ring_n >= (unsigned)CPP) rescore_ring();
            XP(xp_re = wall_clock64(); xp[1] += xp_re - xp_a;)
        }
        if (ring_n > 0u) rescore_ring();
        if (lane == 0) atomicAdd(g.stats + 1, n_cand);
        if (lane == 0) atomicAdd(g.stats + 5, n_entries);
        if (lane == 0 && wave == 0) atomicAdd(reinterpret_cast<unsigned long long*>(g.stats + 2), (unsigned long long)(hend - (own_b - own_a)) * (unsigned long long)(UT / kUserTile));
    }
    __builtin_amdgcn_fence(__ATOMIC_ACQ_REL, "workgroup");
    __syncthreads();
    XP(const unsigned long long xp_e0 = wall_clock64();)
    {
        constexpr int EB = 8;
        uint64_t* scr = crings + wave * kRing5;
        auto emit_row = [&](int rb, int cnt, uint64_t kraw) __attribute__((always_inline)) {
            const int c = min(__builtin_amdgcn_readfirstlane(cnt), CAPL);
            const uint64_t key = lane < c ? kraw : (uint64_t)(63 - lane);
            scr[lane] = key;
            pda_wave_sync();
            int rank = 0;
            for (int jj = 0; jj < c; jj += 4) {
                const uint64_t k0 = scr[jj], k1 = scr[jj + 1], k2 = scr[jj + 2], k3 = scr[jj + 3];
                rank += ((k0 > key) ? 1 : 0) + ((k1 > key) ? 1 : 0) + ((k2 > key) ? 1 : 0) + ((k3 > key) ? 1 : 0);
            }
            pda_wave_sync();
            uint64_t* orow = g.out_keys + ((size_t)split * g.n_users_blk + rb) * K;
            if (lane < c && rank < K) orow[rank] = key;
            if (lane >= c && lane < K) orow[lane] = 0ull;
        };
        if (warm_final) {
            for (int w = 0; w < UPW / 32; ++w) {
                unsigned m = touched[wave * (UPW / 32) + w];
                while (m != 0u) {
                    const int b = __builtin_ctz(m);
                    m &= m - 1u;
                    const int rr = wave * UPW + 32 * w + b;
                    emit_row(utile * UT + rr, cntl[rr], lists[(size_t)rr * CAPL + (lane < CAPL ? lane : CAPL - 1)]);
                }
            }
        } else if (starts_empty) {
            const int rb0 = utile * UT + wave * UPW, nv = max(0, min(UPW, g.n_users_blk - rb0));
            uint64_t* ob = g.out_keys + ((size_t)split * g.n_users_blk + rb0) * K;
            for (int i = lane; i < nv * K; i += 64) ob[i] = 0ull;
            __builtin_amdgcn_fence(__ATOMIC_RELEASE, "workgroup");
            for (int w = 0; w < UPW / 32; ++w) {
                unsigned m = touched[wave * (UPW / 32) + w];
                while (m != 0u) {
                    const int b = __builtin_ctz(m);
                    m &= m - 1u;
                    const int rr = wave * UPW + 32 * w + b;
                    emit_row(utile * UT + rr, cntl[rr], lists[(size_t)rr * CAPL + (lane < CAPL ? lane : CAPL - 1)]);
                }
            }
        } else {
            for (int i0 = 0; i0 < UPW; i0 += EB) {
                uint64_t kraw[EB];
                int cv[EB];
#pragma unroll
                for (int q = 0; q < EB; ++q) {
                    const int rr = wave * UPW + i0 + q, rb = utile * UT + rr;
                    const bool ok = rb < g.n_users_blk;
                    kraw[q] = ok ? lists[(size_t)rr * CAPL + (lane < CAPL ? lane : CAPL - 1)] : 0ull;
                    cv[q] = ok ? cntl[rr] : 0;
                }
#pragma unroll
                for (int q = 0; q < EB; ++q) {
                    const int rb = utile * UT + wave * UPW + i0 + q;
                    if (rb >= g.n_users_blk) break;
                    emit_row(rb, cv[q], kraw[q]);
                }
            }
        }
    }
    XP(xp[7] = wall_clock64() - xp_e0; xp[11] = hend;)
    {
        unsigned n_ent2 = 0, n_ran = 0, n_chunks_other = 0, n_ran_other = 0;
        bool steal = my_rec != nullptr;
        XP(if (pda_v5_tail_pieces > 0) { steal = false; tail_fixed = (own_b - own_a + (unsigned)pda_v5_tail_pieces - 1u) / (unsigned)pda_v5_tail_pieces; })
        const bool others_first = steal && g.tail_others_first != 0;
        bool own_left = own_a < own_b;
        __syncthreads();
        for (;;) {
            unsigned vb = blockIdx.x, a = own_a, b = own_b;
            if (my_rec == nullptr) {
                own_a = own_b;
            } else {
                bool got = false;
                if (others_first) {
                    got = next_chunk(false, false, vb, a, b);
                    if (!got && own_left) { got = next_chunk(true, false, vb, a, b); own_left = got; }
                } else {
                    if (own_left) { got = next_chunk(true, n_ent2 == 0u, vb, a, b); own_left = got; }
                    if (!got && steal) got = next_chunk(false, false, vb, a, b);
                }
                if (!got) a = b = 0;
            }
            if (a >= b) break;
            const int vsplit = (int)(vb % (unsigned)g.n_splits), vutile = (int)(vb / (unsigned)g.n_splits);
            const unsigned vt0 = (unsigned)(vsplit + warm_tiles_of(g, vsplit) * g.n_splits);
            const unsigned char* vfrag = g.ufrag + ((size_t)vutile * 4 + wave) * (size_t)(NU * NK * 1024);
            const size_t vimg = (size_t)g.rows5;
            ++n_ent2;
            n_ran += b - a;
            if (vb != blockIdx.x) { ++n_chunks_other; n_ran_other += b - a; }
            unsigned is = a;
            Loop6Free<D, NU>::run(a, is, b, ring_lds, 1024u * (unsigned)wave, vt0, (unsigned)g.n_splits, (unsigned)vimg, (unsigned)(vimg >> 32), vfrag, lane16);
        }
        if (lane == 0 && n_ent2 > 0u) atomicAdd(g.stats + 5, n_ent2);
        if (lane == 0 && wave == 0 && n_ran > 0u) {
            atomicAdd(g.stats + 7, n_ran);
            atomicAdd(reinterpret_cast<unsigned long long*>(g.stats + 2), (unsigned long long)n_ran * (unsigned long long)(UT / kUserTile));
        }
        if (lane == 0 && wave == 0 && n_chunks_other > 0u) {
            atomicAdd(g.stats + 9, n_chunks_other);
            atomicAdd(g.stats + 10, n_ran_other);
        }
        XP(xp[10] = n_ran_other;)
    }
    XP(xp[5] = wall_clock64() - xp_k0;
       if (lane == 0 && blockIdx.x < (unsigned)kXpMaxWg) for (int q = 0; q < kXpWords; ++q) pda_v5_exitprof[((size_t)blockIdx.x * 4 + wave) * kXpWords + q] = xp[q];)
}

template <int D, bool BF, bool S16, int UPW>
int launch_sweep5(const Args4& g, const Call4& c, hipStream_t stream) {
    constexpr int UT = 4 * UPW;
    constexpr size_t lds = (size_t)kNSlot5 * slot_bytes5(D) + (size_t)UT * 8 + 4 * kRing5 * 8 + (80 + 4) * 4 + 64;
    static_assert(UPW == 256 || D == 256 || 2 * lds <= 160 * 1024, "two workgroups per CU");
    static_assert(lds <= 160 * 1024, "LDS per workgroup");
    static char attr_done[kMaxDev4] = {};
    if (const int rc = dynamic_lds_once(reinterpret_cast<const void*>(&sweep5_kernel<D, BF, S16, UPW>), lds, attr_done)) return rc;
    const int utiles = (g.n_users_blk + UT - 1) / UT, n_pad = utiles * UT;
    if (c.uprep5) {
        hipLaunchKernelGGL((uprep5_kernel<D, BF, S16, UPW>), dim3((unsigned)(((size_t)n_pad * (D / 8) + 255) / 256)), dim3(256), 0, stream, g.U, g.users, g.n_users_blk, n_pad,
                           const_cast<unsigned char*>(g.ufrag), const_cast<float*>(g.unorm));
        PDA_CHECK_LAUNCH();
    }
    hipLaunchKernelGGL((sweep5_kernel<D, BF, S16, UPW>), dim3((unsigned)(utiles * g.n_splits)), dim3(256), lds, stream, g);
    PDA_CHECK_LAUNCH();
    return PDA_OK;
}
```

pda_amd/dist.py:

```python
from __future__ import annotations

from typing import Callable, Iterable, Iterator, Optional, Tuple

import torch
import torch.distributed as dist


def shard_range(n_items: int, rank: int, world: int) -> Tuple[int, int]:
    tiles = (n_items + 31) // 32
    per = ((tiles + world - 1) // world) * 32
    lo = min(rank * per, n_items)
    return lo, min(lo + per, n_items)


def grid_layout(rank: int, world: int, user_groups: int):
    if user_groups < 1 or world % user_groups != 0:
        raise ValueError("world size must be a multiple of the number of user groups")
    per = world // user_groups
    g = rank // per
    return g, rank % per, list(range(g * per, (g + 1) * per))


def default_user_groups(world: int) -> int:
    import os
# ... 99 lines not shown
        if pop_full is None:
            if self.pop_shard is not None:
                self._pop_epoch = getattr(self, "_pop_epoch", 0) + 1
            self.pop_shard, self._pop_src, self._pop_full = None, None, None
            return
        src = getattr(self, "_pop_src", None)
        if src is not None and src[0]() is pop_full and src[1] == pop_full._version and self.pop_shard is not None:
            return
        if pop_full.numel() < self.item_offset + n:
            raise ValueError("popularity vector has %d entries, this shard needs items up to %d" % (pop_full.numel(), self.item_offset + n))
        self.pop_shard = pop_full[self.item_offset:self.item_offset + n].contiguous()
        self._pop_full = pop_full
        self._pop_epoch = getattr(self, "_pop_epoch", 0) + 1
        import weakref
        self._pop_src = (weakref.ref(pop_full), pop_full._version)

    def _seed_reduce(self, bounds):
        self.n_collectives += 1
        dist.all_reduce(bounds, op=dist.ReduceOp.MAX, group=self.group)

    def _seed_sum(self, counts):
        self.n_collectives += 1
        dist.all_reduce(counts, op=dist.ReduceOp.SUM, group=self.group)

    @staticmethod
    def _deep(K) -> bool:
        from . import ops
        return K > ops.TOPK_K_V4

    def _merge(self, K):
        if self._deep(K) and self.merge_fn is _ops_merge_fn():
            from . import ops
            return ops.deep_merge
        return self.merge_fn

    def _seed_applies(self, K, head) -> bool:
        from . import ops
        if self._deep(K):
            return False
        return self.world > 1 and self.seeded and ops.seed_exchange_applies(self.I_shard.shape[1], K, head, self.prune)

    def _validate_once(self, head):
        key = (head, getattr(self, "_pop_epoch", 0))
        if getattr(self, "_validated", None) == key:
            return
        err = ""
        if self.I_shard.shape[0] > (1 << 26):
            err = "seeded item-sharded evaluation: at most 2^26 item rows per shard"
        elif head and self.pop_shard is None and self.I_shard.shape[0] > 0:
            err = "the popularity head needs a popularity vector"
        elif head and self.pop_shard is not None and self.pop_shard.numel() and bool((self.pop_shard < 0).any()):
            err = "pop_shard must be >= 0 (it is pop**gamma of a normalised count)"
        flag = torch.tensor([1.0 if err else 0.0], dtype=torch.float32, device=self.U.device)
        dist.all_reduce(flag, op=dist.ReduceOp.MAX, group=self.group)
        if float(flag[0]) != 0.0:
            raise ValueError(err or "another rank of the item group rejected its shard (see its message)")
        self._validated = key

    def _empty_shard_seed(self, users, K):
        from . import ops
        nu, dev = users.numel(), users.device
        b = torch.empty((3, nu), dtype=torch.float32, device=dev)
        b[0:2] = float("-inf")
        b[2] = float("inf")
        self._seed_reduce(b)
        n_thr = ops.seed_thresholds(self.world)
        if n_thr > 0:
            self._seed_sum(torch.zeros((n_thr, nu), dtype=torch.int32, device=dev))

    def _deep_local_keys(self, users, K, head, hist):
        if self.score_fn is _ops_score_fn():
            from . import ops
            if self.world > 1:
                self._validate_once(head)
            keys = ops.deep_shard_keys(self.U, self.I_shard, users, K, head, self.pop_shard if head else None, hist, self.item_offset)
            return keys[None] if self.world == 1 else keys
        if self.I_shard.shape[0] == 0:
            return torch.zeros((users.numel(), K) if self.world > 1 else (1, users.numel(), K), dtype=torch.int64, device=users.device)
        keys = self.score_fn(self.U, self.I_shard, users, K, head, self.pop_shard if head else None, hist, self.item_offset, 0)
        if self.world == 1:
            return keys
        return keys[0] if keys.shape[0] == 1 else self.merge_fn(keys, users, hist, want="keys")

    def local_keys(self, users, K, head, hist):
        if self._deep(K):
            return self._deep_local_keys(users, K, head, hist)
        seeded = self._seed_applies(K, head)
        if seeded:
            self._validate_once(head)
        if self.I_shard.shape[0] == 0:
            if seeded:
                self._empty_shard_seed(users, K)
            return torch.zeros((users.numel(), K) if self.world > 1 else (1, users.numel(), K), dtype=torch.int64, device=users.device)
        extra = {} if self.prune is None else {"prune": self.prune}
        if seeded:
            extra["seed_reduce"], extra["seed_shards"], extra["seed_sum"] = self._seed_reduce, self.world, self._seed_sum
        keys = self.score_fn(self.U, self.I_shard, users, K, head, self.pop_shard if head else None, hist,
                             self.item_offset, 0, **extra)
        if self.world == 1:
            return keys
        return self.merge_fn(keys, users, hist, want="keys")

    def topk(self, users, K=50, head=0, hist=None):
        keys = self.local_keys(users, K, head, hist)
        if self.world > 1:
            if self._deep(K):
                return self._finish_deep(keys, users, hist, False)
            self.n_collectives += 1
            keys = _all_gather_keys(keys, self.world, self.group)
        return self._merge(K)(keys, users, hist, want="idx_val")

    def user_slice(self, n_users: int) -> Tuple[int, int]:
        per = n_users // self.world
        return self.rank * per, (self.rank + 1) * per

    def _finish(self, keys, users, hist, sharded: bool):
        if self._deep(keys.shape[1]):
            return self._finish_deep(keys, users, hist, sharded)
        self.n_collectives += 1
        if sharded and users.numel() % self.world == 0 and (hist is None or getattr(hist, "mode", 1) == 1):
            lo, hi = self.user_slice(users.numel())
            allk = _exchange_user_slices(keys, self.world, self.group)
            return self.merge_fn(allk, users[lo:hi].contiguous(), hist, want="idx_val")
        allk = _all_gather_keys(keys, self.world, self.group)
        res = self.merge_fn(allk, users, hist, want="idx_val")
        if sharded:
            per = -(-users.numel() // self.world)
            lo = min(self.rank * per, users.numel())
            return tuple(t[lo:lo + per] for t in res)
        return res

    @staticmethod
    def _hist_rows(hist, a, b):
        if hist is None or isinstance(hist, tuple) or getattr(hist, "mode", 1) == 1:
            return hist
        return type(hist)(hist.indptr[a:b + 1].contiguous(), hist.indices, by_user=False)

    def _finish_deep(self, keys, users, hist, sharded: bool):
        nu, K = users.numel(), keys.shape[1]
        merge, chunk, outs = self._merge(K), deep_exchange_chunk(users.numel(), keys.shape[1], self.world), []
        a2a = sharded and nu % self.world == 0 and (hist is None or getattr(hist, "mode", 1) == 1)
        if a2a:
            per, step = nu // self.world, chunk // self.world
            lo, _ = self.user_slice(nu)
            by_owner = keys.view(self.world, per, K)
            for a in range(0, per, step):
                b = min(per, a + step)
                self.n_collectives += 1
                allk = _exchange_user_slices(by_owner[:, a:b].reshape(-1, K), self.world, self.group)
                outs.append(merge(allk, users[lo + a:lo + b].contiguous(), hist, want="idx_val"))
        else:
            for a in range(0, nu, chunk):
                b = min(nu, a + chunk)
                self.n_collectives += 1
                allk = _all_gather_keys(keys[a:b], self.world, self.group)
                outs.append(merge(allk, users[a:b].contiguous(), self._hist_rows(hist, a, b), want="idx_val"))
        res = outs[0] if len(outs) == 1 else tuple(torch.cat(t) for t in zip(*outs))
        if sharded and not a2a:
            per = -(-nu // self.world)
            lo = min(self.rank * per, nu)
            return tuple(t[lo:lo + per] for t in res)
        return res

    def topk_sharded(self, users, K=50, head=0, hist=None):
        keys = self.local_keys(users, K, head, hist)
        if self.world == 1:
            return self._merge(K)(keys, users, hist, want="idx_val")
        return self._finish(keys, users, hist, True)

    def _hot_applies(self, K, head, hist, users, sharded) -> bool:
        if self._deep(K):
            return False
        if not (self.hot_items and self.world >= 2 and sharded and head == 1 and self.prune in ("order", True, None)):
            return False
        if self.world < self.hot_min_shards and users.numel() < self.hot_min_users_two_shards:
            return False
        if getattr(self, "_pop_full", None) is None or users.numel() % self.world != 0:
            return False
        if hist is not None and getattr(hist, "mode", 1) != 1:
            return False
        fns = self._hot_fns()
        if fns is None or self._pop_full.numel() < 4 * self.hot_items:
            return False
        if self.sweep_seed_fn is not None and self.kth_fn is not None:
            return True
        from . import ops
        d = int(self.U.shape[1])
        return d in (64, 128, 256) and K <= ops.TOPK_K_V4

    def _hot_fns(self):
        if self.sweep_seed_fn is not None and self.kth_fn is not None:
            return self.sweep_seed_fn, self.kth_fn
        if self.score_fn is _ops_score_fn():
            from . import ops
            return ops.sweep_from_seed, ops.kth_value
        return None

    def _hot_state(self):
        key = (getattr(self, "_pop_epoch", 0), self.I_shard._version, self.hot_items)
        if self._hot is not None and self._hot["key"] == key:
            return self._hot
        pop_full, lo, n, dev = self._pop_full, self.item_offset, self.I_shard.shape[0], self.I_shard.device
        H = self.hot_items
        hot_ids = torch.argsort(pop_full, descending=True, stable=True)[:H].sort().values
        mine = (hot_ids >= lo) & (hot_ids < lo + n)
        hot_I = torch.zeros((H, self.I_shard.shape[1]), dtype=self.I_shard.dtype, device=dev)
        if n > 0:
            hot_I[mine] = self.I_shard[hot_ids[mine] - lo]
        self.n_epoch_collectives += 1
        if hot_I.dtype == torch.bfloat16:
            t = hot_I.float()
            dist.all_reduce(t, op=dist.ReduceOp.SUM, group=self.group)
            hot_I = t.to(torch.bfloat16)
        else:
            dist.all_reduce(hot_I, op=dist.ReduceOp.SUM, group=self.group)
        cold_mask = torch.ones(n, dtype=torch.bool, device=dev)
        if n > 0:
            cold_mask[hot_ids[mine] - lo] = False
        cold_local = torch.nonzero(cold_mask).flatten()
        st = {"key": key, "hot_ids": hot_ids, "hot_I": hot_I.contiguous(), "hot_pop": pop_full[hot_ids].contiguous(),
              "hot_gid": hot_ids.to(torch.int32),
              "I_cold": self.I_shard[cold_local].contiguous(), "pop_cold": self.pop_shard[cold_local].contiguous(),
              "cold_gid": (cold_local + lo).to(torch.int32), "cold_index_of": torch.cumsum(cold_mask, 0) - 1, "hist": None}
        self._hot = st
        return st

    def _hot_hist(self, st, hist):
        if hist is None:
            return None, None
        if st["hist"] is not None and st["hist"][0] is hist:
            return st["hist"][1], st["hist"][2]
        as_tuple = isinstance(hist, tuple)
        indptr = torch.as_tensor(hist[0]) if as_tuple else hist.indptr
        indices = torch.as_tensor(hist[1]) if as_tuple else hist.indices
        dev, n_rows = indices.device, indptr.numel() - 1
        hot_ids, lo, n = st["hot_ids"].to(dev), self.item_offset, self.I_shard.shape[0]
        rows = torch.repeat_interleave(torch.arange(n_rows, device=dev), indptr[1:] - indptr[:-1])
        idx = indices.long()
        pos = torch.searchsorted(hot_ids, idx).clamp_(max=hot_ids.numel() - 1)
        is_hot = hot_ids[pos] == idx
        loc = idx - lo
        is_cold = (loc >= 0) & (loc < n) & ~is_hot

        def csr(sel, local_ids):
            ptr = torch.zeros(n_rows + 1, dtype=torch.int64, device=dev)
            torch.cumsum(torch.bincount(rows[sel], minlength=n_rows), 0, out=ptr[1:])
            ix = local_ids.to(torch.int32).contiguous()
            if as_tuple:
# ... 349 lines not shown
```

pda_amd/ops.py:

```python
from __future__ import annotations

import math
import os
from typing import Optional, Tuple

import ctypes as C

import torch

from . import _lib
from ._lib import (HEAD_POP, HEAD_RAW, HIST_BY_BLOCK_ROW, HIST_BY_USER_ID, UPD_ANY_ORDER, UPD_DENSE_GRAD, UPD_NONE, UPD_USERS_DISTINCT,
                   UPD_SGD_FUSED, check, ptr, stream_ptr)

ADAM_BETA1, ADAM_BETA2, ADAM_EPS = 0.9, 0.999, 1e-8


def _need(t: Optional[torch.Tensor], dtype, name: str, optional=False):
    if t is None:
        if optional:
            return None
        raise ValueError(f"{name} is required")
    if not t.is_cuda:
        raise ValueError(f"{name} must live in HBM (cuda tensor); pda_amd has no CPU path")
    if t.dtype != dtype:
# ... 386 lines not shown

def remap_key_items(keys: torch.Tensor, gid: torch.Tensor) -> torch.Tensor:
    keys = _need(keys, torch.int64, "keys")
    gid = _need(gid, torch.int32, "gid")
    check(_lib.load().pda_topk_remap_items(ptr(keys), keys.numel(), ptr(gid), gid.numel(), stream_ptr()), "pda_topk_remap_items")
    return keys


def sweep_from_seed(U, I_shard, users, K, head, pop_shard, hist, item_offset, seed: torch.Tensor, n_splits: int = 0, prune="order",
                    stats: Optional[dict] = None) -> torch.Tensor:
    lib = _lib.load()
    bf = I_shard.dtype == torch.bfloat16
    U = _need(U, torch.bfloat16 if bf else torch.float32, "U")
    I_shard = _need(I_shard, torch.bfloat16 if bf else torch.float32, "I_shard")
    users = _need(users, torch.int32, "users")
    seed = _need(seed, torch.float32, "seed")
    pop_shard = _need(pop_shard, torch.float32, "pop_shard", optional=True)
    nu, nloc, d = users.numel(), I_shard.shape[0], I_shard.shape[1]
    if seed.numel() != nu:
        raise ValueError("seed must have one entry per user of the block")
    if d not in (64, 128, 256) or K > TOPK_K_V4:
        raise ValueError("sweep_from_seed: embed dim 64/128/256 and K <= %d" % TOPK_K_V4)
    if head == HEAD_POP and pop_shard is not None:
        _check_pop(pop_shard)
    if hist is not None and hist.indices.numel() == 0:
        hist = None
    order = visiting_order(I_shard, pop_shard if head == HEAD_POP else None) if prune else None
    prep = item_prep4(I_shard, pop_shard if head == HEAD_POP else None, order)
    if n_splits <= 0:
        n_splits = lib.pda_score_topk4_auto_splits(nu, nloc, d)
        if head == HEAD_POP and prune == "order" and d in (64, 128, 256) and not os.environ.get("PDA_SCORE_LISTS") and pop_shard is not None:
            n_splits = huge_splits(nu, nloc, d) or n_splits
    out = torch.empty((n_splits, nu, K), dtype=torch.int64, device=U.device)
    ws = torch.empty(lib.pda_score_topk4_workspace_bytes(nu, nloc, d, n_splits), dtype=torch.uint8, device=U.device)
    es = (1 if prune is True else 0) | few_candidates_hint(head, prune, nu, d, nloc, n_splits)
    fn = lib.pda_score_topk4_phase_bf16 if bf else lib.pda_score_topk4_phase_f32
    check(fn(ptr(U), ptr(I_shard), ptr(prep), ptr(pop_shard), ptr(users), nu, item_offset, nloc, d,
             ptr(hist.indptr) if hist else None, ptr(hist.indices) if hist else None, hist.mode if hist else 0, K, head, es, n_splits,
             4, 0, ptr(seed), ptr(out), ptr(ws), stream_ptr()), "pda_score_topk4_phase (sweep from a seed)")
    if os.environ.get("PDA_CHECK_SWEEP_ERRORS"):
        err = int(ws[0:4].view(torch.int32)[0])
        if err != 0:
            raise RuntimeError("pda_score_topk4_phase: the sweep reported protocol error %d" % err)
    if stats is not None:
        stats["pairs_rescored"] = ws[4:8].view(torch.int32)
        stats["kernel_id"] = ws[16:20].view(torch.int32)
        stats["huge_entries"] = ws[20:24].view(torch.int32)
        stats["huge_free_halftiles"] = ws[28:32].view(torch.int32)
        stats["error"] = ws[0:4].view(torch.int32)
    return out


def tail_record_offset(nu: int) -> int:
    return (_lib.load().pda_score_topk_workspace_bytes(nu) + 255) & ~255


def seeded_counts(c: SeededCall) -> Optional[torch.Tensor]:
    if c.n_thr <= 0:
        return None
    c.counts = torch.empty((c.n_thr, c.nu), dtype=torch.int32, device=c.bounds.device)
    check(c.lib.pda_topk_seed_counts(ptr(c.out), c.n_splits, c.nu, c.K, ptr(c.bounds), c.n_thr, ptr(c.counts), stream_ptr()),
          "pda_topk_seed_counts")
    return c.counts


def seeded_finish(c: SeededCall) -> torch.Tensor:
    seed = torch.empty(c.nu, dtype=torch.float32, device=c.bounds.device)
    check(c.lib.pda_topk_seed_pick(ptr(c.bounds), ptr(c.counts), c.n_thr if c.counts is not None else 0, c.nu, c.K, ptr(seed), stream_ptr()),
          "pda_topk_seed_pick")
    check(c.fnp(*c.common, 2, c.wt, ptr(seed), ptr(c.out), ptr(c.ws), stream_ptr()), "pda_score_topk4_phase (sweep)")
    if c.stats is not None:
        c.stats["tiles_scored"] = c.ws[8:16].view(torch.int64)
        c.stats["pairs_rescored"] = c.ws[4:8].view(torch.int32)
        c.stats["tiles_dense"] = ((c.nloc + 31) // 32) * ((c.nu + 127) // 128)
        c.stats["kernel_id"] = c.ws[16:20].view(torch.int32)
        c.stats["error"] = c.ws[0:4].view(torch.int32)
    out, c.keep = c.out, None
    return out


def score_topk_keys(U, I_shard, users, K=50, head=HEAD_RAW, pop_shard=None, hist: Optional[HistoryCSR] = None,
                    item_offset=0, n_splits=0, out: Optional[torch.Tensor] = None, impl: Optional[str] = None,
                    prune=None, stats: Optional[dict] = None, seed_reduce=None, seed_shards: int = 1, seed_sum=None,
                    warm_tiles: int = 0) -> torch.Tensor:
    lib = _lib.load()
    bf = I_shard is not None and I_shard.dtype == torch.bfloat16
    U = _need(U, torch.bfloat16 if bf else torch.float32, "U")
    I_shard = _need(I_shard, torch.bfloat16 if bf else torch.float32, "I_shard")
    users = _need(users, torch.int32, "users")
    pop_shard = _need(pop_shard, torch.float32, "pop_shard", optional=True)
    nu, nloc, d = users.numel(), I_shard.shape[0], I_shard.shape[1]
    if bf:
        if d not in (64, 128, 256) or K > TOPK_CAP_V2 or impl == "v1":
            raise ValueError("bf16 tables: embed dim 64/128/256, K <= %d, no v1 entry point" % TOPK_CAP_V2)
        impl = "v2"
    if U.shape[1] != d:
        raise ValueError("U and I_shard disagree on embed dim")
    if pop_shard is not None and pop_shard.numel() != nloc:
        raise ValueError("pop_shard must have one entry per local item row")
    if head == HEAD_POP and pop_shard is not None:
        _check_pop(pop_shard)
    if hist is not None and hist.indices.numel() == 0:
        hist = None
    n_splits_auto = n_splits <= 0
    out_given = out
    impl = impl or score_impl(d, K, item_offset + nloc)
    if prune is None:
        prune = prune_default(head, d)
    if seed_reduce is not None and seed_exchange_applies(d, K, head, prune, impl):
        if out_given is not None:
            raise ValueError("the seeded sweep allocates its own output")
        c = seeded_begin(U, I_shard, users, K, head, pop_shard, hist, item_offset, n_splits, seed_shards, stats=stats)
        seed_reduce(c.bounds)
        cnt = seeded_counts(c) if seed_sum is not None else None
        if cnt is not None:
            seed_sum(cnt)
        return seeded_finish(c)
    if n_splits_auto and out_given is None and impl == "v2" and funnel_applies(d, K, nu, nloc, head, prune, hist):
        return score_topk_funnel(U, I_shard, users, K, hist, item_offset, stats)
    if n_splits <= 0:
        n_splits = lib.pda_score_topk_auto_splits(nu, nloc)
    if out is None:
        out = torch.empty((n_splits, nu, K), dtype=torch.int64, device=U.device)
    elif out.shape != (n_splits, nu, K) or out.dtype != torch.int64:
        raise ValueError("out must be int64 [n_splits, Bu, K]")
    if impl == "v2" and score_kernel(d, K, nloc, prune, head) == "v4":
        order = visiting_order(I_shard, pop_shard if head == HEAD_POP else None) if prune else None
        prep = item_prep4(I_shard, pop_shard if head == HEAD_POP else None, order)
        forced_env = any(os.environ.get(k) for k in ("PDA_SCORE_LISTS", "PDA_SCORE_KERNEL", "PDA_HUGE_SPLITS"))
        plan = None
        if n_splits_auto and out_given is None and not forced_env and not (head == HEAD_POP and pop_shard is None):
            plan = score_plan(nu, nloc, d, K, head, prune, bf, hist)
            if plan["kernel"] != "v4":
                plan = None
        if plan is not None:
            n_splits = plan["n_splits"]
            out = torch.empty((n_splits, nu, K), dtype=torch.int64, device=U.device)
        elif n_splits_auto and out_given is None:
            n_splits = lib.pda_score_topk4_auto_splits(nu, nloc, d)
            if head == HEAD_POP and prune == "order" and d in (64, 128, 256) and not os.environ.get("PDA_SCORE_LISTS") and pop_shard is not None:
                n_splits = huge_splits(nu, nloc, d) or n_splits
            out = torch.empty((n_splits, nu, K), dtype=torch.int64, device=U.device)
        ws = torch.empty(lib.pda_score_topk4_workspace_bytes(nu, nloc, d, n_splits), dtype=torch.uint8, device=U.device)
        hint = plan["early_stop"] if plan is not None else ((1 if prune is True else 0) | few_candidates_hint(head, prune, nu, d, nloc, n_splits))
        es = hint | ((min(4, max(0, int(warm_tiles))) & 7) << 4)
        if os.environ.get("PDA_WARM_PER_SPLIT"):
            es |= SWEEP_WARM_PER_SPLIT
        if os.environ.get("PDA_WARM_ONE_KERNEL"):
            es |= SWEEP_WARM_ONE_KERNEL
        if os.environ.get("PDA_SWEEP_TAIL_SHARE") == "0":
            es |= SWEEP_TAIL_NO_SHARE
        if os.environ.get("PDA_SWEEP_TAIL_OTHERS_FIRST"):
            es |= SWEEP_TAIL_OTHERS_FIRST
        if os.environ.get("PDA_SWEEP_TAIL_MIN_CHUNK") == "2":
            es |= SWEEP_TAIL_MIN2
        tab = warm_mask_table(hist, prep, order, item_offset, nloc, d) if hist and (n_splits == 1 or not (es & SWEEP_WARM_PER_SPLIT)) else None
        if tab is not None:
            fn = lib.pda_score_topk4_phase_masked_bf16 if bf else lib.pda_score_topk4_phase_masked_f32
            check(fn(ptr(U), ptr(I_shard), ptr(prep), ptr(pop_shard), ptr(users), nu, item_offset, nloc, d,
                     ptr(hist.indptr), ptr(hist.indices), hist.mode, K, head, es, n_splits, ptr(tab), tab.shape[0],
                     ptr(out), ptr(ws), stream_ptr()), "pda_score_topk4_phase_masked")
        else:
            fn = lib.pda_score_topk4_bf16 if bf else lib.pda_score_topk4_f32
            check(fn(ptr(U), ptr(I_shard), ptr(prep), ptr(pop_shard), ptr(users), nu, item_offset, nloc, d,
                     ptr(hist.indptr) if hist else None, ptr(hist.indices) if hist else None, hist.mode if hist else 0,
                     K, head, es, n_splits, ptr(out), ptr(ws), stream_ptr()), "pda_score_topk4")
        if os.environ.get("PDA_CHECK_SWEEP_ERRORS"):
            err = int(ws[0:4].view(torch.int32)[0])
            if err != 0:
                raise RuntimeError("pda_score_topk4: the sweep reported protocol error %d" % err)
        if stats is not None:
            stats["tiles_scored"] = ws[8:16].view(torch.int64)
            stats["pairs_rescored"] = ws[4:8].view(torch.int32)
            stats["tiles_dense"] = ((nloc + 31) // 32) * ((nu + 127) // 128)
            stats["kernel_id"] = ws[16:20].view(torch.int32)
            stats["huge_entries"] = ws[20:24].view(torch.int32)
            stats["huge_free_halftiles"] = ws[28:32].view(torch.int32)
            stats["warm_kernels"] = ws[32:36].view(torch.int32)
            stats["tail_stolen_chunks"] = ws[36:40].view(torch.int32)
            stats["tail_stolen_halftiles"] = ws[40:44].view(torch.int32)
            stats["tail_records"] = ws[tail_record_offset(nu):tail_record_offset(nu) + 8 * (-(-nu // (512 if d == 256 else 1024)) * n_splits)].view(torch.int64)
            stats["error"] = ws[0:4].view(torch.int32)
            stats["workspace"] = ws
            stats["n_splits"] = n_splits
            stats["warm_mask_table"] = tab
        return out
    if impl == "v2" and prune:
        prep, order = item_prep_ordered(I_shard, pop_shard if head == HEAD_POP else None)
        hist_ord = hist_reordered(hist, prep, order, item_offset, nloc, d) if hist else None
        ws = torch.empty(lib.pda_score_topk_workspace_bytes(nu), dtype=torch.uint8, device=U.device)
        fn = lib.pda_score_topk_ordered_bf16 if bf else lib.pda_score_topk_ordered_f32
        check(fn(ptr(U), ptr(I_shard), ptr(prep), ptr(pop_shard), ptr(users), nu, item_offset,
                                             nloc, d, ptr(hist.indptr) if hist else None,
                                             ptr(hist.indices) if hist else None, ptr(hist_ord), hist.mode if hist else 0,
                                             K, head, 0 if prune == "order" else 1, n_splits, ptr(out), ptr(ws), stream_ptr()),
              "pda_score_topk_ordered")
        if stats is not None:
            stats["tiles_scored"] = ws[8:16].view(torch.int64)
            stats["pairs_rescored"] = ws[4:8].view(torch.int32)
            stats["tiles_dense"] = ((nloc + 31) // 32) * ((nu + 127) // 128)
            stats["kernel_id"] = ws[16:20].view(torch.int32)
        return out
    if impl == "v2":
        prep = item_prep(I_shard)
        ws = torch.empty(lib.pda_score_topk_workspace_bytes(nu), dtype=torch.uint8, device=U.device)
        fn = lib.pda_score_topk_bf16 if bf else lib.pda_score_topk_prepped_f32
        check(fn(ptr(U), ptr(I_shard), ptr(prep), ptr(pop_shard), ptr(users), nu, item_offset,
                                             nloc, d, ptr(hist.indptr) if hist else None,
                                             ptr(hist.indices) if hist else None, hist.mode if hist else 0, K, head,
                                             n_splits, ptr(out), ptr(ws), stream_ptr()), "pda_score_topk_prepped_f32")
        return out
    check(lib.pda_score_topk_f32(ptr(U), ptr(I_shard), ptr(pop_shard), ptr(users), nu, item_offset, nloc, d,
                                 ptr(hist.indptr) if hist else None, ptr(hist.indices) if hist else None,
                                 hist.mode if hist else 0, K, head, n_splits, ptr(out), stream_ptr()),
          "pda_score_topk_f32")
    return out


FUNNEL_MIN_USERS = 1
FUNNEL_MIN_ITEMS = 4096
FUNNEL_BLOCK_ROW_MAX_USERS = 16384
FUNNEL_SMALL_ITEMS, FUNNEL_SMALL_MAX_USERS = 20000, 16384
_FUNNEL_ORDER = {}


def funnel_order(I_shard: torch.Tensor) -> torch.Tensor:
    key = (I_shard.shape[0], str(I_shard.device))
    o = _FUNNEL_ORDER.get(key)
    if o is None:
        g = torch.Generator(device="cpu").manual_seed(0x5EED + I_shard.shape[0])
        o = torch.randperm(I_shard.shape[0], generator=g).to(torch.int32).to(I_shard.device)
        _FUNNEL_ORDER[key] = o
    return o


FUNNEL_WORKSPACE_BUDGET = 24 << 30


def funnel_applies(d: int, K: int, nu: int, nloc: int, head: int, prune, hist: Optional[HistoryCSR]) -> bool:
    can = head == HEAD_RAW and d in (64, 128, 256) and K <= TOPK_K_V4 and 4096 <= nloc <= (1 << 26) and prune is not True \
        and (hist is None or hist.mode == HIST_BY_USER_ID or nu <= FUNNEL_BLOCK_ROW_MAX_USERS)
    forced = os.environ.get("PDA_SCORE_FUNNEL", "")
    if forced == "0" or not can:
        return False
    if forced == "1":
        return True
    return nu >= FUNNEL_MIN_USERS and nloc >= FUNNEL_MIN_ITEMS and (nloc >= FUNNEL_SMALL_ITEMS or nu <= FUNNEL_SMALL_MAX_USERS) \
        and not os.environ.get("PDA_SCORE_KERNEL") and not os.environ.get("PDA_SCORE_LISTS") \
        and _lib.load().pda_score_topk7_workspace_bytes(nu, nloc, d) <= FUNNEL_WORKSPACE_BUDGET


def score_topk_funnel(U, I_shard, users, K=50, hist: Optional[HistoryCSR] = None, item_offset=0, stats: Optional[dict] = None) -> torch.Tensor:
    lib = _lib.load()
    bf = I_shard.dtype == torch.bfloat16
    U = _need(U, torch.bfloat16 if bf else torch.float32, "U")
    I_shard = _need(I_shard, torch.bfloat16 if bf else torch.float32, "I_shard")
    users = _need(users, torch.int32, "users")
    nu, nloc, d = users.numel(), I_shard.shape[0], I_shard.shape[1]
    if hist is not None and hist.indices.numel() == 0:
        hist = None
    prep = item_prep7(I_shard, funnel_order(I_shard))
# ... 3163 lines not shown
```

Baseline: 34.97 million users/s.

## Write final top-K index/value lists directly from the sweep kernel

Adds a LISTS variant of the sweep5 kernel and the warm/select paths that write int32 item ids and float scores straight into the output arrays, instead of emitting packed 64-bit keys that a separate merge/unpack pass converts later. Short rows are padded from the user's history inside the kernel, and a NaN-tagged kth value carries the short count. The goal is to remove the extra unpack kernel and the round trip of the key buffer for the single-GPU, single-split, huge-geometry pop-head case. In exchange it adds more template instantiations and per-row serial fill logic in the epilogue.

```diff
diff --git a/include/pda_hip_experimental.h b/include/pda_hip_experimental.h
--- a/include/pda_hip_experimental.h
+++ b/include/pda_hip_experimental.h
@@ -43,6 +43,15 @@
                                     const int64_t* hist_indptr, const int32_t* hist_indices, int hist_row_mode, int warm_tiles, uint32_t* out,
                                     void* stream);
 int pda_score_topk4_phase_mask_offsets(int n_users_blk, int n_items_local, int d, int n_splits, size_t* offs);
+int pda_score_topk4_phase_lists_apply(int n_users_blk, int n_items_local, int d, int K, int head, int early_stop, int n_splits);
+int pda_score_topk4_phase_lists_f32(const float* U, const float* I_shard, const void* prep, const float* pop_shard, const int32_t* users,
+                                    int n_users_blk, int item_offset, int n_items_local, int d, const int64_t* hist_indptr,
+                                    const int32_t* hist_indices, int hist_row_mode, int K, int head, int early_stop, int n_splits,
+                                    const uint32_t* mask_table, int mask_table_rows, int32_t* out_idx, float* out_val, void* workspace, void* stream);
+int pda_score_topk4_phase_lists_bf16(const uint16_t* U, const uint16_t* I_shard, const void* prep, const float* pop_shard, const int32_t* users,
+                                     int n_users_blk, int item_offset, int n_items_local, int d, const int64_t* hist_indptr,
+                                     const int32_t* hist_indices, int hist_row_mode, int K, int head, int early_stop, int n_splits,
+                                     const uint32_t* mask_table, int mask_table_rows, int32_t* out_idx, float* out_val, void* workspace, void* stream);
 int pda_score_topk7_phase_user_image(const void* U, int bf16, const int32_t* users, int n_users_blk, int d, void* ufrag, float* unorm, float* uerr,
                                      void* stream);
 int pda_score_topk4_phase_bloom_rows(const void* prep, const int32_t* users, int n_users_blk, const int64_t* hist_indptr,
diff --git a/pda_amd/_lib.py b/pda_amd/_lib.py
--- a/pda_amd/_lib.py
+++ b/pda_amd/_lib.py
@@ -85,6 +85,9 @@
     "pda_score_topk7_phase_bloom_rows": (_i, [_vp, _vp, _i, _i, _i, _i, _vp, _vp, _i, _vp, _vp]),
     "pda_score_topk4_phase_masked_f32": (_i, [_vp, _vp, _vp, _vp, _vp, _i, _i, _i, _i, _vp, _vp, _i, _i, _i, _i, _i, _vp, _i, _vp, _vp, _vp]),
     "pda_score_topk4_phase_masked_bf16": (_i, [_vp, _vp, _vp, _vp, _vp, _i, _i, _i, _i, _vp, _vp, _i, _i, _i, _i, _i, _vp, _i, _vp, _vp, _vp]),
+    "pda_score_topk4_phase_lists_apply": (_i, [_i, _i, _i, _i, _i, _i, _i]),
+    "pda_score_topk4_phase_lists_f32": (_i, [_vp, _vp, _vp, _vp, _vp, _i, _i, _i, _i, _vp, _vp, _i, _i, _i, _i, _i, _vp, _i, _vp, _vp, _vp, _vp]),
+    "pda_score_topk4_phase_lists_bf16": (_i, [_vp, _vp, _vp, _vp, _vp, _i, _i, _i, _i, _vp, _vp, _i, _i, _i, _i, _i, _vp, _i, _vp, _vp, _vp, _vp]),
     "pda_score_topk_plan": (_i, [_i, _i, _i, _i, _i, _i, _i, _i, _vp]),
     "pda_score_topk_huge_splits": (_i, [_i, _i, _i]),
     "pda_score_topk7_workspace_bytes": (_sz, [_i, _i, _i]),
diff --git a/pda_amd/csrc/pda_score_topk_v4.hip b/pda_amd/csrc/pda_score_topk_v4.hip
--- a/pda_amd/csrc/pda_score_topk_v4.hip
+++ b/pda_amd/csrc/pda_score_topk_v4.hip
@@ -74,7 +74,29 @@
     uint64_t* tail_rec;
     unsigned tail_min;
     int tail_others_first;
+    int32_t* out_idx;
+    float* out_val;
 };
+
+__device__ __forceinline__ int32_t list_id(uint64_t k) { return pda_key_item(k); }
+__device__ __forceinline__ float list_val(uint64_t k) { return (uint32_t)(k >> 32) != 0u ? pda_key_val(k) : -INFINITY; }
+__device__ __forceinline__ uint64_t list_key(int32_t id, float v) { return (id == -1 && v == -INFINITY) ? 0ull : pda_pack_key(v, (uint32_t)id); }
+__device__ __forceinline__ float kth_short(int c) { return __uint_as_float(0x7FC00000u | (uint32_t)c); }
+__device__ __forceinline__ bool kth_is_short(float kth, int& c) {
+    const uint32_t b = __float_as_uint(kth);
+    if ((b & 0x7FFFFFFFu) <= 0x7F800000u) return false;
+    c = (int)(b & 0xFFFFu);
+    return true;
+}
+__device__ __forceinline__ void fill_short_row(const Args4& g, int rb, int c, uint64_t* row) {
+    const int64_t hr = g.hist_row_mode == PDA_HIST_BY_USER_ID ? (int64_t)g.users[rb] : (int64_t)rb;
+    int fill = c, prev = -1;
+    for (int64_t p = g.hist_indptr[hr]; p < g.hist_indptr[hr + 1] && fill < g.K; ++p) {
+        const int it = g.hist_indices[p];
+        if (it != prev) row[fill++] = (uint64_t)(0xFFFFFFFFu - (uint32_t)it);
+        prev = it;
+    }
+}
 
 struct Call4 {
     enum Warm { kNoWarm, kWarm4, kWarmTwo };
@@ -716,16 +738,38 @@
         const int rb0 = utile * kUserTile + wave * 32, nv = max(0, min(32, g.n_users_blk - rb0));
         if (lane < nv) {
             const uint64_t kl = my_lists[(size_t)lane * CAP + (K - 1)];
-            g.kth_ws[(size_t)split * g.n_users_blk + rb0 + lane] = cntl[wave * 32 + lane] >= K ? pda_unordf((uint32_t)(kl >> 32)) : -INFINITY;
-        }
-        uint64_t* ob = g.out_keys + ((size_t)split * g.n_users_blk + rb0) * K;
+            const int cl = cntl[wave * 32 + lane];
+            g.kth_ws[(size_t)split * g.n_users_blk + rb0 + lane] = cl >= K ? pda_unordf((uint32_t)(kl >> 32)) : g.out_idx != nullptr ? kth_short(cl) : -INFINITY;
+        }
         const int q64 = 64 / K, r64 = 64 % K;
         int rr = lane / K, p = lane % K;
-        for (int i = lane; i < nv * K; i += 64) {
-            ob[i] = p < cntl[wave * 32 + rr] ? my_lists[(size_t)rr * CAP + p] : 0ull;
-            rr += q64;
-            p += r64;
-            if (p >= K) { p -= K; ++rr; }
+        if (g.out_idx != nullptr) {
+            for (int r = 0; r < nv; ++r) {
+                const int c = __builtin_amdgcn_readfirstlane(cntl[wave * 32 + r]);
+                if (c >= K) continue;
+                if (lane >= c && lane < K) my_lists[(size_t)r * CAP + lane] = 0ull;
+                pda_wave_sync();
+                if (g.hist_indptr != nullptr && lane == 0) fill_short_row(g, rb0 + r, c, my_lists + (size_t)r * CAP);
+            }
+            pda_wave_sync();
+            int32_t* oi = g.out_idx + (size_t)rb0 * K;
+            float* ov = g.out_val + (size_t)rb0 * K;
+            for (int i = lane; i < nv * K; i += 64) {
+                const uint64_t k = my_lists[(size_t)rr * CAP + p];
+                oi[i] = list_id(k);
+                ov[i] = list_val(k);
+                rr += q64;
+                p += r64;
+                if (p >= K) { p -= K; ++rr; }
+            }
+        } else {
+            uint64_t* ob = g.out_keys + ((size_t)split * g.n_users_blk + rb0) * K;
+            for (int i = lane; i < nv * K; i += 64) {
+                ob[i] = p < cntl[wave * 32 + rr] ? my_lists[(size_t)rr * CAP + p] : 0ull;
+                rr += q64;
+                p += r64;
+                if (p >= K) { p -= K; ++rr; }
+            }
         }
     }
     if (g.pred_ws != nullptr && lane < 32) {
@@ -1039,20 +1083,52 @@
         for (int s = 0; s < 2; ++s)
             if (lane < cs[s]) lists[wave][s][rank[s]] = key[s];
         pda_wave_sync();
-#pragma unroll
-        for (int s = 0; s < 2; ++s) {
-            const int rb = rb0 + it + s;
-            if (rb < n) {
-                if (lane < K) g.out_keys[(size_t)rb * K + lane] = lists[wave][s][lane];
-                const uint64_t kl = lists[wave][s][K - 1];
-                if (lane == it + s) kth_mine = cs[s] >= K ? pda_unordf((uint32_t)(kl >> 32)) : -INFINITY;
+        if (g.out_idx != nullptr) {
+            const int nrow = min(2, n - (rb0 + it));
+            if (g.hist_indptr != nullptr && (cs[0] < K || (nrow > 1 && cs[1] < K))) {
+                if (lane == 0) {
+                    if (cs[0] < K) fill_short_row(g, rb0 + it, cs[0], lists[wave][0]);
+                    if (nrow > 1 && cs[1] < K) fill_short_row(g, rb0 + it + 1, cs[1], lists[wave][1]);
+                }
+                pda_wave_sync();
+            }
+            typedef int32_t i32x2 __attribute__((ext_vector_type(2)));
+            typedef float f32x2 __attribute__((ext_vector_type(2)));
+            const size_t o0 = (size_t)(rb0 + it) * K;
+            const int e0 = 2 * lane, ne = nrow * K;
+            if (e0 < ne) {
+                const uint64_t ka = lists[wave][0][e0 < K ? e0 : 64 + (e0 - K)];
+                if (e0 + 1 < ne) {
+                    const uint64_t kb = lists[wave][0][e0 + 1 < K ? e0 + 1 : 64 + (e0 + 1 - K)];
+                    const i32x2 iv = {list_id(ka), list_id(kb)};
+                    const f32x2 vv = {list_val(ka), list_val(kb)};
+                    *reinterpret_cast<i32x2*>(g.out_idx + o0 + e0) = iv;
+                    *reinterpret_cast<f32x2*>(g.out_val + o0 + e0) = vv;
+                } else {
+                    g.out_idx[o0 + e0] = list_id(ka);
+                    g.out_val[o0 + e0] = list_val(ka);
+                }
+            }
+#pragma unroll
+            for (int s = 0; s < 2; ++s)
+                if (lane == it + s) kth_mine = cs[s] >= K ? pda_key_val(lists[wave][s][K - 1]) : kth_short(cs[s]);
+        } else {
+#pragma unroll
+            for (int s = 0; s < 2; ++s) {
+                const int rb = rb0 + it + s;
+                if (rb < n) {
+                    if (lane < K) g.out_keys[(size_t)rb * K + lane] = lists[wave][s][lane];
+                    const uint64_t kl = lists[wave][s][K - 1];
+                    if (lane == it + s) kth_mine = cs[s] >= K ? pda_unordf((uint32_t)(kl >> 32)) : -INFINITY;
+                }
             }
         }
         pda_wave_sync();
     }
     if (lane < kSelRows && rb0 + lane < n) {
         g.kth_ws[rb0 + lane] = kth_mine;
-        if (g.seed_out != nullptr) g.seed_out[rb0 + lane] = kth_mine;
+        int c_short;
+        if (g.seed_out != nullptr) g.seed_out[rb0 + lane] = kth_is_short(kth_mine, c_short) ? -INFINITY : kth_mine;
     }
 }
 
@@ -2110,12 +2186,19 @@
     return ws4_layout(n_users_blk, d, n_splits).total;
 }
 
+static bool lists_call4(bool huge_hint, int head, int early_stop_bit, int n_tiles, int n_splits, int warm_tiles, int n_users_blk, int K) {
+    return huge_hint && head == PDA_HEAD_POP && !early_stop_bit && n_splits == 1 && n_tiles > warm_tiles && (uint64_t)n_users_blk * (uint64_t)K <= (1ull << 30);
+}
+
 int run_score4(const void* U, const void* I_shard, bool bf16, const void* prep, const float* pop_shard, const int32_t* users,
                int n_users_blk, int item_offset, int n_items_local, int d, const int64_t* hist_indptr, const int32_t* hist_indices,
                int hist_row_mode, int K, int head, int early_stop, int n_splits, uint64_t* out_keys, void* workspace, hipStream_t s,
                int phase = 3, const float* seed = nullptr, int warm_tiles = 0, const int* n_users_dev = nullptr,
-               const uint32_t* mask_table = nullptr, int mask_table_rows = 0) {
-    if (!U || !I_shard || !prep || !users || !out_keys || !workspace) return PDA_ERR_ARG;
+               const uint32_t* mask_table = nullptr, int mask_table_rows = 0, int32_t* out_idx = nullptr, float* out_val = nullptr) {
+    const bool lists = out_idx != nullptr || out_val != nullptr;
+    if (lists && (!out_idx || !out_val || out_keys)) return PDA_ERR_ARG;
+    if (lists && ((reinterpret_cast<uintptr_t>(out_idx) | reinterpret_cast<uintptr_t>(out_val)) & 7u) != 0) return PDA_ERR_ARG;
+    if (!U || !I_shard || !prep || !users || (!out_keys && !lists) || !workspace) return PDA_ERR_ARG;
     if (n_users_blk <= 0 || n_items_local <= 0 || item_offset < 0) return PDA_ERR_ARG;
     if (K < 1 || K > PDA_MAX_K) return PDA_ERR_ARG;
     if (early_stop < 0 || (early_stop & ~0x7FFF) != 0) return PDA_ERR_ARG;
@@ -2155,6 +2238,8 @@
               : (geometry == 3 && d <= 128) ? Call4::kSweep4Many : Call4::kSweep4;
     const bool dense5 = phase == 3 && c.sweep == Call4::kSweep5 && !c.ends_in_warm;
     c.uprep5 = !(dense5 && n_users_dev == nullptr);
+    if (lists && !(dense5 && lists_call4(geometry == 4, head, early_stop, L.n_tiles, n_splits, warm_tiles, n_users_blk, K) && seed == nullptr && n_users_dev == nullptr))
+        return PDA_ERR_UNSUPPORTED;
     const bool warm_shared = phase == 3 && n_splits > 1 && seed == nullptr && !warm_per_split && L.n_tiles > n_splits * warm_tiles;
     c.warm_whole = n_splits == 1 || warm_shared;
     c.warm = !(phase & 1) ? Call4::kNoWarm
@@ -2176,6 +2261,8 @@
     g.hist_indptr = hist_indptr;
     g.hist_indices = hist_indices;
     g.out_keys = out_keys;
+    g.out_idx = out_idx;
+    g.out_val = out_val;
     g.rows = pb + L.rows;
     g.sufA = early_stop ? reinterpret_cast<const float*>(pb + L.sufA) : nullptr;
     g.sufB = early_stop ? reinterpret_cast<const float*>(pb + (pop_head ? L.sufB : L.sufR)) : nullptr;
@@ -2511,6 +2598,34 @@
                       mask_table, mask_table_rows);
 }
 
+extern "C" int pda_score_topk4_phase_lists_apply(int n_users_blk, int n_items_local, int d, int K, int head, int early_stop, int n_splits) {
+    if (n_users_blk <= 0 || n_items_local <= 0 || (d != 64 && d != 128 && d != 256) || K < 1 || K > kCap4 - 3) return 0;
+    if (early_stop < 0 || (early_stop & ~0x7FFF) != 0 || (uint64_t)n_items_local > (1ull << 26)) return 0;
+    int warm_tiles = (early_stop >> 4) & 7;
+    if (warm_tiles > kWarmTiles) return 0;
+    if (warm_tiles == 0) warm_tiles = kWarmTiles;
+    if (n_splits <= 0) n_splits = pda_score_topk4_auto_splits(n_users_blk, n_items_local, d);
+    return lists_call4((early_stop & PDA_SWEEP_HUGE) != 0, head, early_stop & 1, prep4_layout(n_items_local, d).n_tiles, n_splits, warm_tiles, n_users_blk, K) ? 1 : 0;
+}
+extern "C" int pda_score_topk4_phase_lists_f32(const float* U, const float* I_shard, const void* prep, const float* pop_shard, const int32_t* users,
+                                               int n_users_blk, int item_offset, int n_items_local, int d, const int64_t* hist_indptr,
+                                               const int32_t* hist_indices, int hist_row_mode, int K, int head, int early_stop, int n_splits,
+                                               const uint32_t* mask_table, int mask_table_rows, int32_t* out_idx, float* out_val, void* workspace, void* stream) {
+    if (!out_idx || !out_val || (mask_table != nullptr && mask_table_rows <= 0)) return PDA_ERR_ARG;
+    return run_score4(U, I_shard, false, prep, pop_shard, users, n_users_blk, item_offset, n_items_local, d, hist_indptr, hist_indices,
+                      hist_row_mode, K, head, early_stop, n_splits, nullptr, workspace, reinterpret_cast<hipStream_t>(stream), 3, nullptr, 0, nullptr,
+                      mask_table, mask_table_rows, out_idx, out_val);
+}
+extern "C" int pda_score_topk4_phase_lists_bf16(const uint16_t* U, const uint16_t* I_shard, const void* prep, const float* pop_shard, const int32_t* users,
+                                                int n_users_blk, int item_offset, int n_items_local, int d, const int64_t* hist_indptr,
+                                                const int32_t* hist_indices, int hist_row_mode, int K, int head, int early_stop, int n_splits,
+                                                const uint32_t* mask_table, int mask_table_rows, int32_t* out_idx, float* out_val, void* workspace, void* stream) {
+    if (!out_idx || !out_val || (mask_table != nullptr && mask_table_rows <= 0)) return PDA_ERR_ARG;
+    return run_score4(U, I_shard, true, prep, pop_shard, users, n_users_blk, item_offset, n_items_local, d, hist_indptr, hist_indices,
+                      hist_row_mode, K, head, early_stop, n_splits, nullptr, workspace, reinterpret_cast<hipStream_t>(stream), 3, nullptr, 0, nullptr,
+                      mask_table, mask_table_rows, out_idx, out_val);
+}
+
 static Args4 mask_args4(const void* prep, const int32_t* users, int n_rows, int item_offset, int n_items_local, int d, const int64_t* hist_indptr,
                         const int32_t* hist_indices, int hist_row_mode, int warm_tiles) {
     const Prep4Layout L = prep4_layout(n_items_local, d);
diff --git a/pda_amd/csrc/pda_v5_sweep.h b/pda_amd/csrc/pda_v5_sweep.h
--- a/pda_amd/csrc/pda_v5_sweep.h
+++ b/pda_amd/csrc/pda_v5_sweep.h
@@ -19,7 +19,7 @@
 
 
 
-template <int D, bool BF, bool S16, int UPW>
+template <int D, bool BF, bool S16, int UPW, bool LISTS = false>
 __global__ void __launch_bounds__(256, 1) sweep5_kernel(Args4 g) {
     static_assert(slot_bytes5(D) == Loop6<D, 8>::kSlotBytes, "one LDS image for all loops");
     static_assert(S16, "the loop on v_mfma_f32_32x32x16_bf16 (round 4's first form: 9.16 against 8.07 ms, profiles/README.md) left with round 5; the parameter keeps the kernel's name");
@@ -51,6 +51,7 @@
     const unsigned hend = 2u * (unsigned)n_it;
     if (tid < 72) sync[tid] = (tid < 8 || tid >= 40 || warm_final || starts_empty) ? 0u : 0xFFFFFFFFu;
     if (tid == 0 && blockIdx.x == 0) g.stats[4] = (4u << 28) | (4u << 8) | (1u << 13) | ((BF ? 1u : 0u) << 14) | (unsigned)(D >> 6);
+    if (LISTS && tid == 0 && blockIdx.x == 0) g.stats[11] = 1u;
     if (starts_empty) {
         for (int rr = tid; rr < UT; rr += 256) {
             cntl[rr] = 0;
@@ -65,7 +66,9 @@
             if (rb < g.n_users_blk) {
                 tau = g.kth_ws[(size_t)split * g.n_users_blk + rb];
                 c = K;
-                if (tau == -INFINITY) {
+                if constexpr (LISTS) {
+                    if (kth_is_short(tau, c)) tau = -INFINITY;
+                } else if (tau == -INFINITY) {
                     const uint64_t* row = g.out_keys + ((size_t)split * g.n_users_blk + rb) * K;
                     for (c = 0; c < K && row[c] != 0ull; ++c) {}
                 }
@@ -297,7 +300,12 @@
                             const int lr = row0 + __builtin_amdgcn_readlane(row, __builtin_ctzll(need));
                             need &= need - 1ull;
                             const int c_r = cntl[lr];
-                            if (lane < c_r) lists[(size_t)lr * CAPL + lane] = g.out_keys[((size_t)split * g.n_users_blk + (size_t)(utile * UT + lr)) * K + lane];
+                            if constexpr (LISTS) {
+                                const unsigned o = (unsigned)(utile * UT + lr) * (unsigned)K + (unsigned)lane;
+                                if (lane < c_r) lists[(size_t)lr * CAPL + lane] = list_key(g.out_idx[o], g.out_val[o]);
+                            } else if (lane < c_r) {
+                                lists[(size_t)lr * CAPL + lane] = g.out_keys[((size_t)split * g.n_users_blk + (size_t)(utile * UT + lr)) * K + lane];
+                            }
                         }
                         list_sync<true>();
                     }
@@ -519,6 +527,32 @@
             if (lane < c && rank < K) orow[rank] = key;
             if (lane >= c && lane < K) orow[lane] = 0ull;
         };
+        auto emit_row_lists = [&](int rb, int cnt, uint64_t kraw) __attribute__((always_inline)) {
+            const int c = min(__builtin_amdgcn_readfirstlane(cnt), CAPL);
+            const uint64_t key = lane < c ? kraw : (uint64_t)(63 - lane);
+            uint64_t* fin = scr + 64;
+            scr[lane] = key;
+            pda_wave_sync();
+            int rank = 0;
+            for (int jj = 0; jj < c; jj += 4) {
+                const uint64_t k0 = scr[jj], k1 = scr[jj + 1], k2 = scr[jj + 2], k3 = scr[jj + 3];
+                rank += ((k0 > key) ? 1 : 0) + ((k1 > key) ? 1 : 0) + ((k2 > key) ? 1 : 0) + ((k3 > key) ? 1 : 0);
+            }
+            if (lane < c && rank < K) fin[rank] = key;
+            if (lane >= c && lane < K) fin[lane] = 0ull;
+            pda_wave_sync();
+            if (c < K && g.hist_indptr != nullptr) {
+                if (lane == 0) fill_short_row(g, rb, c, fin);
+                pda_wave_sync();
+            }
+            if (lane < K) {
+                const uint64_t k = fin[lane];
+                const unsigned o = (unsigned)rb * (unsigned)K + (unsigned)lane;
+                g.out_idx[o] = list_id(k);
+                g.out_val[o] = list_val(k);
+            }
+            pda_wave_sync();
+        };
         if (warm_final) {
             for (int w = 0; w < UPW / 32; ++w) {
                 unsigned m = touched[wave * (UPW / 32) + w];
@@ -526,7 +560,9 @@
                     const int b = __builtin_ctz(m);
                     m &= m - 1u;
                     const int rr = wave * UPW + 32 * w + b;
-                    emit_row(utile * UT + rr, cntl[rr], lists[(size_t)rr * CAPL + (lane < CAPL ? lane : CAPL - 1)]);
+                    const uint64_t kraw = lists[(size_t)rr * CAPL + (lane < CAPL ? lane : CAPL - 1)];
+                    if constexpr (LISTS) emit_row_lists(utile * UT + rr, cntl[rr], kraw);
+                    else emit_row(utile * UT + rr, cntl[rr], kraw);
                 }
             }
         } else if (starts_empty) {
@@ -612,21 +648,24 @@
        if (lane == 0 && blockIdx.x < (unsigned)kXpMaxWg) for (int q = 0; q < kXpWords; ++q) pda_v5_exitprof[((size_t)blockIdx.x * 4 + wave) * kXpWords + q] = xp[q];)
 }
 
-template <int D, bool BF, bool S16, int UPW>
+template <int D, bool BF, bool S16, int UPW, bool LISTS = false>
 int launch_sweep5(const Args4& g, const Call4& c, hipStream_t stream) {
+    if constexpr (!LISTS) {
+        if (g.out_idx != nullptr) return launch_sweep5<D, BF, S16, UPW, true>(g, c, stream);
+    }
     constexpr int UT = 4 * UPW;
     constexpr size_t lds = (size_t)kNSlot5 * slot_bytes5(D) + (size_t)UT * 8 + 4 * kRing5 * 8 + (80 + 4) * 4 + 64;
     static_assert(UPW == 256 || D == 256 || 2 * lds <= 160 * 1024, "two workgroups per CU");
     static_assert(lds <= 160 * 1024, "LDS per workgroup");
     static char attr_done[kMaxDev4] = {};
-    if (const int rc = dynamic_lds_once(reinterpret_cast<const void*>(&sweep5_kernel<D, BF, S16, UPW>), lds, attr_done)) return rc;
+    if (const int rc = dynamic_lds_once(reinterpret_cast<const void*>(&sweep5_kernel<D, BF, S16, UPW, LISTS>), lds, attr_done)) return rc;
     const int utiles = (g.n_users_blk + UT - 1) / UT, n_pad = utiles * UT;
     if (c.uprep5) {
         hipLaunchKernelGGL((uprep5_kernel<D, BF, S16, UPW>), dim3((unsigned)(((size_t)n_pad * (D / 8) + 255) / 256)), dim3(256), 0, stream, g.U, g.users, g.n_users_blk, n_pad,
                            const_cast<unsigned char*>(g.ufrag), const_cast<float*>(g.unorm));
         PDA_CHECK_LAUNCH();
     }
-    hipLaunchKernelGGL((sweep5_kernel<D, BF, S16, UPW>), dim3((unsigned)(utiles * g.n_splits)), dim3(256), lds, stream, g);
+    hipLaunchKernelGGL((sweep5_kernel<D, BF, S16, UPW, LISTS>), dim3((unsigned)(utiles * g.n_splits)), dim3(256), lds, stream, g);
     PDA_CHECK_LAUNCH();
     return PDA_OK;
 }
diff --git a/pda_amd/dist.py b/pda_amd/dist.py
--- a/pda_amd/dist.py
+++ b/pda_amd/dist.py
@@ -205,7 +205,7 @@
             return keys
         return keys[0] if keys.shape[0] == 1 else self.merge_fn(keys, users, hist, want="keys")
 
-    def local_keys(self, users, K, head, hist):
+    def local_keys(self, users, K, head, hist, lists_out=None):
         if self._deep(K):
             return self._deep_local_keys(users, K, head, hist)
         seeded = self._seed_applies(K, head)
@@ -218,14 +218,22 @@
         extra = {} if self.prune is None else {"prune": self.prune}
         if seeded:
             extra["seed_reduce"], extra["seed_shards"], extra["seed_sum"] = self._seed_reduce, self.world, self._seed_sum
+        if lists_out is not None:
+            extra["lists_out"] = lists_out
         keys = self.score_fn(self.U, self.I_shard, users, K, head, self.pop_shard if head else None, hist,
                              self.item_offset, 0, **extra)
         if self.world == 1:
             return keys
         return self.merge_fn(keys, users, hist, want="keys")
 
+    def _lists_holder(self, K):
+        return {} if self.world == 1 and not self._deep(K) and self.merge_fn is _ops_merge_fn() else None
+
     def topk(self, users, K=50, head=0, hist=None):
-        keys = self.local_keys(users, K, head, hist)
+        holder = self._lists_holder(K)
+        keys = self.local_keys(users, K, head, hist, holder)
+        if holder:
+            return holder["idx"], holder["val"]
         if self.world > 1:
             if self._deep(K):
                 return self._finish_deep(keys, users, hist, False)
@@ -286,7 +294,10 @@
         return res
 
     def topk_sharded(self, users, K=50, head=0, hist=None):
-        keys = self.local_keys(users, K, head, hist)
+        holder = self._lists_holder(K)
+        keys = self.local_keys(users, K, head, hist, holder)
+        if holder:
+            return holder["idx"], holder["val"]
         if self.world == 1:
             return self._merge(K)(keys, users, hist, want="idx_val")
         return self._finish(keys, users, hist, True)
diff --git a/pda_amd/ops.py b/pda_amd/ops.py
--- a/pda_amd/ops.py
+++ b/pda_amd/ops.py
@@ -492,7 +492,7 @@
 def score_topk_keys(U, I_shard, users, K=50, head=HEAD_RAW, pop_shard=None, hist: Optional[HistoryCSR] = None,
                     item_offset=0, n_splits=0, out: Optional[torch.Tensor] = None, impl: Optional[str] = None,
                     prune=None, stats: Optional[dict] = None, seed_reduce=None, seed_shards: int = 1, seed_sum=None,
-                    warm_tiles: int = 0) -> torch.Tensor:
+                    warm_tiles: int = 0, lists_out: Optional[dict] = None) -> Optional[torch.Tensor]:
     lib = _lib.load()
     bf = I_shard is not None and I_shard.dtype == torch.bfloat16
     U = _need(U, torch.bfloat16 if bf else torch.float32, "U")
@@ -565,7 +565,19 @@
         if os.environ.get("PDA_SWEEP_TAIL_MIN_CHUNK") == "2":
             es |= SWEEP_TAIL_MIN2
         tab = warm_mask_table(hist, prep, order, item_offset, nloc, d) if hist and (n_splits == 1 or not (es & SWEEP_WARM_PER_SPLIT)) else None
-        if tab is not None:
+        by_writers = (lists_out is not None and out_given is None and n_splits == 1 and not os.environ.get("PDA_LISTS_BY_UNPACK")
+                      and lib.pda_score_topk4_phase_lists_apply(nu, nloc, d, K, head, es, n_splits) == 1)
+        if by_writers:
+            out = None
+            idx = torch.empty((nu, K), dtype=torch.int32, device=U.device)
+            val = torch.empty((nu, K), dtype=torch.float32, device=U.device)
+            fn = lib.pda_score_topk4_phase_lists_bf16 if bf else lib.pda_score_topk4_phase_lists_f32
+            check(fn(ptr(U), ptr(I_shard), ptr(prep), ptr(pop_shard), ptr(users), nu, item_offset, nloc, d,
+                     ptr(hist.indptr) if hist else None, ptr(hist.indices) if hist else None, hist.mode if hist else 0, K, head, es, n_splits,
+                     ptr(tab) if tab is not None else None, tab.shape[0] if tab is not None else 0,
+                     ptr(idx), ptr(val), ptr(ws), stream_ptr()), "pda_score_topk4_phase_lists")
+            lists_out["idx"], lists_out["val"] = idx, val
+        elif tab is not None:
             fn = lib.pda_score_topk4_phase_masked_bf16 if bf else lib.pda_score_topk4_phase_masked_f32
             check(fn(ptr(U), ptr(I_shard), ptr(prep), ptr(pop_shard), ptr(users), nu, item_offset, nloc, d,
                      ptr(hist.indptr), ptr(hist.indices), hist.mode, K, head, es, n_splits, ptr(tab), tab.shape[0],
@@ -587,6 +599,7 @@
             stats["huge_entries"] = ws[20:24].view(torch.int32)
             stats["huge_free_halftiles"] = ws[28:32].view(torch.int32)
             stats["warm_kernels"] = ws[32:36].view(torch.int32)
+            stats["lists_by"] = ws[44:48].view(torch.int32)
             stats["tail_stolen_chunks"] = ws[36:40].view(torch.int32)
             stats["tail_stolen_halftiles"] = ws[40:44].view(torch.int32)
             stats["tail_records"] = ws[tail_record_offset(nu):tail_record_offset(nu) + 8 * (-(-nu // (512 if d == 256 else 1024)) * n_splits)].view(torch.int64)
```

New measurement: 35.00 million users/s, median of 2. About the same (+0.1%).
